# thomaspingel/neilpy

Hardware: AMD Instinct MI355X
Metric: Mcells/s through SMRF progressive_filter, 16384x16384 fp32 DEM (higher is better)
Workload: dtype f32

## Files before the change

### neilpy_amd/build.py

```python
import argparse
import os
import shutil
import subprocess
import sys
from concurrent.futures import ThreadPoolExecutor

PKG = os.path.dirname(os.path.abspath(__file__))
ROOT = os.path.dirname(PKG)
CSRC = os.path.join(PKG, "csrc")
OBJ = os.path.join(PKG, "_build")
LIBDIR = os.path.join(PKG, "_lib")
LIB = os.path.join(LIBDIR, "libsmrf_hip.so")
RING_PARTS = 8

FLAGS = ["-std=c++20", "-O3", "--offload-arch=gfx950", "-fPIC", "-ffp-contract=off",
         "-fvisibility=hidden", "-Wall", "-Wno-unused-function",
         "-I" + os.path.join(ROOT, "include"), "-I" + CSRC]


def hipcc():
    exe = shutil.which("hipcc") or "/opt/rocm/bin/hipcc"
    if not os.path.exists(exe):
        raise RuntimeError("hipcc not found: libsmrf_hip cannot be built (there is no CPU fallback)")
    return exe


def units():
    out = [(n + ".o", os.path.join(CSRC, n + ".hip"), []) for n in ("core", "morph", "incero", "chain", "grid", "springs", "fda", "tail", "spline", "terrain", "surface", "nearest", "focal", "morphometry", "points", "voxel", "relief", "assign", "footprint", "rank", "label")]
    for f64 in (0, 1):
        for p in range(RING_PARTS):
            out.append(("ring_%s_p%d.o" % ("f64" if f64 else "f32", p), os.path.join(CSRC, "ring_part.hip"),
                        ["-DPART=%d" % p, "-DSMRF_F64=%d" % f64]))
    return out


def newest_header():
    inc = os.path.join(ROOT, "include")
    t = max(os.path.getmtime(os.path.join(inc, f)) for f in os.listdir(inc) if f.endswith(".h"))
    for f in os.listdir(CSRC):
        if f.endswith((".h", ".inc")):
            t = max(t, os.path.getmtime(os.path.join(CSRC, f)))
    return t


def build(jobs=None, force=False, verbose=True, variant=None, defs=()):
    global OBJ, LIB
    if variant:
        OBJ = os.path.join(PKG, "_build", "variant_" + variant)
        LIB = os.path.join(LIBDIR, "variants", variant + ".so")
        os.makedirs(os.path.dirname(LIB), exist_ok=True)
    os.makedirs(OBJ, exist_ok=True)
    os.makedirs(LIBDIR, exist_ok=True)
    cc = hipcc()
    hdr = newest_header()
    todo = []
    objs = []
    for name, src, extra in units():
        obj = os.path.join(OBJ, name)
        objs.append(obj)
        if force or not os.path.exists(obj) or os.path.getmtime(obj) < max(os.path.getmtime(src), hdr):
            todo.append((obj, src, extra))

    def compile_one(job):
        obj, src, extra = job
        cmd = [cc] + FLAGS + list(defs) + extra + ["-c", src, "-o", obj]
        r = subprocess.run(cmd, capture_output=True, text=True)
        if r.returncode != 0:
            raise RuntimeError("hipcc failed: %s\n%s" % (" ".join(cmd), r.stderr[-4000:]))
        if verbose:
            print("  built", os.path.basename(obj), flush=True)
        return obj

    jobs = jobs or min(8, os.cpu_count() or 1)
    if todo:
        if verbose:
            print("compiling %d translation units for gfx950 with %d jobs" % (len(todo), jobs), flush=True)
        with ThreadPoolExecutor(max_workers=jobs) as ex:
            list(ex.map(compile_one, todo))
    if todo or not os.path.exists(LIB):
        cmd = [cc, "-shared", "-fPIC", "--offload-arch=gfx950", "-o", LIB] + objs
        r = subprocess.run(cmd, capture_output=True, text=True)
        if r.returncode != 0:
            raise RuntimeError("link failed: %s\n%s" % (" ".join(cmd), r.stderr[-4000:]))
        if verbose:
            print("linked", LIB, flush=True)
    return LIB


if __name__ == "__main__":
    ap = argparse.ArgumentParser()
    ap.add_argument("-j", type=int, default=None)
    ap.add_argument("--force", action="store_true")
    ap.add_argument("--variant", default=None)
    ap.add_argument("--defs", default="", help="extra compiler flags for a variant build, space separated")
    a = ap.parse_args()
    build(a.j, a.force, variant=a.variant, defs=tuple(a.defs.split()))
    sys.exit(0)
```

### neilpy_amd/csrc/core.hip

```cpp
#include <atomic>
#include <cstring>

#include "smrf_common.h"

namespace {
thread_local char g_err[512] = "";
}

namespace {
int env_int(const char* name, int dflt) {
  const char* v = getenv(name);
  return v && *v ? atoi(v) : dflt;
}
SmrfSwitches read_switches() {
  SmrfSwitches s;
  s.fused = env_int("SMRF_FUSED", 1);
  s.chain = env_int("SMRF_CHAIN", 1);
  s.nan_ride = env_int("SMRF_NAN_RIDE", 1);
  s.nt = env_int("SMRF_NT", -1);
  s.ring_seg = env_int("SMRF_RING_SEG", 0);
  s.ring_dual = env_int("SMRF_RING_DUAL", -1);
  s.ring_rounds = env_int("SMRF_RING_ROUNDS", 1);
  s.ring_slope = env_int("SMRF_RING_SLOPE", -1);
  s.seg_rule = env_int("SMRF_SEG_RULE", 0);
  s.xcd_remap = env_int("SMRF_XCD_REMAP", 1);
  s.fused_rounds = env_int("SMRF_FUSED_ROUNDS", 1);
  s.chain_rounds = env_int("SMRF_CHAIN_ROUNDS", 3);
  s.ring_debug = env_int("SMRF_RING_DEBUG", 0);
  s.ero_inc = env_int("SMRF_ERO_INC", 1);
  s.dil_cross = env_int("SMRF_DIL_CROSS", 1);
  return s;
}
std::atomic<const SmrfSwitches*> g_sw{new SmrfSwitches(read_switches())};
}

const SmrfSwitches& smrf_sw() { return *g_sw.load(std::memory_order_acquire); }

int smrf_fail(int code, const char* fmt, ...) {
  va_list ap;
  va_start(ap, fmt);
  vsnprintf(g_err, sizeof(g_err), fmt, ap);
  va_end(ap);
  return code;
}

extern "C" {

int smrf_abi_version(void) { return SMRF_ABI_VERSION; }

const char* smrf_last_error(void) { return g_err; }

void smrf_switches_reload(void) { g_sw.store(new SmrfSwitches(read_switches()), std::memory_order_release); }

int smrf_device_count(void) {
  int n = 0;
  if (hipGetDeviceCount(&n) != hipSuccess) {
    (void)hipGetLastError();
    return 0;
  }
  return n;
}

}
```

### neilpy_amd/csrc/morph.hip

```cpp
#include <algorithm>
#include <cmath>
#include <cstdlib>
#include <cstring>
#include <vector>

#include "smrf_common.h"
#include "morph_chain.h"

namespace {

template <typename T, bool DIL>
__global__ __launch_bounds__(256) void direct_kernel(const DiskArgs<T> a) {
  const int x = blockIdx.x * 64 + (threadIdx.x & 63);
  const int y = a.out_row0 + blockIdx.y * 4 + (threadIdx.x >> 6);
  if (x >= a.cols || y >= a.out_row0 + a.out_rows) return;
  const int r = a.radius;
  const long long r2 = (long long)r * r;
  T best = DIL ? -INFINITY : INFINITY;
  bool first_nan = false;
  for (int dy = -r; dy <= r; ++dy) {
    const int ly = smrf_fold(y + dy, a.img_rows) - a.in_row0;
    const T* row = a.in + (long long)ly * a.ld;
    long long rem = r2 - (long long)dy * dy;
    int w = (int)sqrt((double)rem);
    while ((long long)(w + 1) * (w + 1) <= rem) ++w;
    while ((long long)w * w > rem) --w;
    for (int dx = -w; dx <= w; ++dx) {
      const T v = row[smrf_fold(x + dx, a.cols)];
      if (dy == -r && dx == 0) first_nan = (v != v);
      if (DIL) { if (v > best) best = v; } else { if (v < best) best = v; }
    }
  }
  if (a.nan_aware && first_nan) best = DIL ? (T)NAN : (T)NAN;
  const long long off = (long long)(y - a.out_row0) * a.ld + x;
  a.out[off] = best;
  if (a.mask != nullptr) smrf::smrf_flag_cell(a, off, a.last[off], best);
}

template <typename T>
__global__ __launch_bounds__(256) void copy_flag_kernel(const DiskArgs<T> a) {
  const long long n = (long long)a.out_rows * a.cols;
  for (long long i = blockIdx.x * 256ll + threadIdx.x; i < n; i += (long long)gridDim.x * 256) {
    const int yy = (int)(i / a.cols), x = (int)(i % a.cols);
    const T v = a.in[(long long)(a.out_row0 + yy - a.in_row0) * a.ld + x];
    const long long off = (long long)yy * a.ld + x;
    a.out[off] = v;
    if (a.mask != nullptr) smrf::smrf_flag_cell(a, off, a.last[off], v);
  }
}

template <typename T>
__global__ __launch_bounds__(256) void count_nan_kernel(const T* __restrict__ p, long long n,
                                                        unsigned long long* __restrict__ out) {
  unsigned long long c = 0;
  for (long long i = blockIdx.x * 256ll + threadIdx.x; i < n; i += (long long)gridDim.x * 256) {
    const T v = p[i];
    c += (v != v);
  }
  for (int o = 32; o > 0; o >>= 1) c += __shfl_down(c, o, 64);
  if ((threadIdx.x & 63) == 0 && c) atomicAdd(out, c);
}

template <typename T> struct RingFn;
template <> struct RingFn<float> {
  static int call(const DiskArgs<float>& a, int d, hipStream_t s) {
    switch (a.radius % SMRF_RING_PARTS) {
      case 0: return smrf_ring_f32_p0(a, d, s);
      case 1: return smrf_ring_f32_p1(a, d, s);
      case 2: return smrf_ring_f32_p2(a, d, s);
      case 3: return smrf_ring_f32_p3(a, d, s);
      case 4: return smrf_ring_f32_p4(a, d, s);
      case 5: return smrf_ring_f32_p5(a, d, s);
      case 6: return smrf_ring_f32_p6(a, d, s);
      default: return smrf_ring_f32_p7(a, d, s);
    }
  }
};
template <> struct RingFn<double> {
  static int call(const DiskArgs<double>& a, int d, hipStream_t s) {
    switch (a.radius % SMRF_RING_PARTS) {
      case 0: return smrf_ring_f64_p0(a, d, s);
      case 1: return smrf_ring_f64_p1(a, d, s);
      case 2: return smrf_ring_f64_p2(a, d, s);
      case 3: return smrf_ring_f64_p3(a, d, s);
      case 4: return smrf_ring_f64_p4(a, d, s);
      case 5: return smrf_ring_f64_p5(a, d, s);
      case 6: return smrf_ring_f64_p6(a, d, s);
      default: return smrf_ring_f64_p7(a, d, s);
    }
  }
};

template <typename T>
int check_band(const DiskArgs<T>& a) {
  if (!a.in || !a.out) return smrf_fail(SMRF_E_ARG, "null raster pointer");
  if (a.img_rows < 1 || a.cols < 1 || a.in_rows < 1 || a.out_rows < 1 || a.radius < 0)
    return smrf_fail(SMRF_E_ARG, "bad raster size (%d x %d, in %d, out %d, radius %d)", a.img_rows,
                     a.cols, a.in_rows, a.out_rows, a.radius);
  if (a.ld < a.cols) return smrf_fail(SMRF_E_ARG, "ld %lld < cols %d", a.ld, a.cols);
  if (a.out_row0 < 0 || a.out_row0 + a.out_rows > a.img_rows || a.in_row0 < 0 ||
      a.in_row0 + a.in_rows > a.img_rows)
    return smrf_fail(SMRF_E_ARG, "row band outside the raster");
  const int lo = a.out_row0 - a.radius, hi = a.out_row0 + a.out_rows + a.radius;
  const int span = hi - lo;
  if (span >= 2 * a.img_rows) {
    if (a.in_row0 != 0 || a.in_rows != a.img_rows)
      return smrf_fail(SMRF_E_ARG, "band must hold the whole raster when radius >= rows");
  } else {
    for (int y = lo; y < hi; ++y) {
      const int g = smrf_fold(y, a.img_rows);
      if (g < a.in_row0 || g >= a.in_row0 + a.in_rows)
        return smrf_fail(SMRF_E_ARG, "input band [%d,%d) lacks row %d needed by output rows [%d,%d) at radius %d",
                         a.in_row0, a.in_row0 + a.in_rows, g, a.out_row0, a.out_row0 + a.out_rows, a.radius);
    }
  }
  return SMRF_OK;
}

template <typename T>
int disk_filter(DiskArgs<T> a, bool dilate, int impl, hipStream_t stream) {
  if (int rc = check_band(a)) return rc;
  if (a.radius == 0) {
    const long long n = (long long)a.out_rows * a.cols;
    const int blocks = (int)std::min<long long>((n + 255) / 256, 4096);
    hipLaunchKernelGGL(copy_flag_kernel<T>, dim3(blocks), dim3(256), 0, stream, a);
    SMRF_LAUNCH_CHECK();
    return SMRF_OK;
  }
  if (impl == SMRF_IMPL_AUTO) impl = a.radius <= SMRF_RING_MAX_RADIUS ? SMRF_IMPL_RING : SMRF_IMPL_DIRECT;
  if (impl == SMRF_IMPL_RING) {
    if (a.radius > SMRF_RING_MAX_RADIUS)
      return smrf_fail(SMRF_E_UNSUPPORTED, "ring kernels cover radius <= %d (got %d)", SMRF_RING_MAX_RADIUS, a.radius);
    a.seg = smrf_sw().ring_seg;
    return RingFn<T>::call(a, dilate ? SMRF_RING_DILATE : SMRF_RING_ERODE, stream);
  }
  if (impl != SMRF_IMPL_DIRECT) return smrf_fail(SMRF_E_ARG, "unknown impl %d", impl);
  dim3 grid((a.cols + 63) / 64, (a.out_rows + 3) / 4);
  if (dilate) hipLaunchKernelGGL((direct_kernel<T, true>), grid, dim3(256), 0, stream, a);
  else hipLaunchKernelGGL((direct_kernel<T, false>), grid, dim3(256), 0, stream, a);
  SMRF_LAUNCH_CHECK();
  return SMRF_OK;
}

template <typename T>
int nt_rule(int img_rows, int cols) {
  const int env = smrf_sw().nt;
  if (env >= 0) return env != 0;
  return (size_t)img_rows * (size_t)cols * sizeof(T) >= ((size_t)192 << 20);
}

template <typename T, template <typename> class Args>
void set_band(Args<T>& a, int img_rows, int cols, int64_t ld, int in_row0, int in_rows, int out_row0, int out_rows) {
  a.img_rows = img_rows; a.cols = cols; a.ld = ld;
  a.in_row0 = in_row0; a.in_rows = in_rows; a.out_row0 = out_row0; a.out_rows = out_rows;
  a.nt = nt_rule<T>(img_rows, cols);
}

template <typename T>
int disk_filter_api(const T* in, T* out, int img_rows, int cols, int64_t ld, int in_row0, int in_rows,
                    int out_row0, int out_rows, int radius, int is_dilate, int nan_aware, int impl, void* stream) {
  DiskArgs<T> a{};
  a.in = in; a.out = out;
  set_band(a, img_rows, cols, ld, in_row0, in_rows, out_row0, out_rows);
  a.radius = radius; a.nan_aware = nan_aware;
  return disk_filter(a, is_dilate != 0, impl, (hipStream_t)stream);
}

template <typename T>
int dilate_flag_api(const T* eroded, const T* last, T* opened, uint8_t* mask, uint8_t* when, double thr,
                    int widx, int img_rows, int cols, int64_t ld, int in_row0, int in_rows, int out_row0,
                    int out_rows, int radius, int nan_aware, int impl, void* stream, int dense = 0) {
  if (!last || !mask) return smrf_fail(SMRF_E_ARG, "null last/mask pointer");
  DiskArgs<T> a{};
  a.in = eroded; a.out = opened; a.last = last; a.mask = mask; a.when = when; a.thr = thr; a.thr_lo = smrf_float_below(thr); a.widx = widx;
  set_band(a, img_rows, cols, ld, in_row0, in_rows, out_row0, out_rows);
  a.radius = radius; a.nan_aware = nan_aware; a.dense = dense;
  return disk_filter(a, true, impl, (hipStream_t)stream);
}

int dilate_cross_flag_f32(const float* e_prev, const float* last, float* opened, uint8_t* mask, uint8_t* when, double thr, int widx,
                          int rows, int cols, int radius, hipStream_t stream) {
  if (!smrf_dil_cross_has(4, radius)) return smrf_fail(SMRF_E_UNSUPPORTED, "no cross-on-load dilation for radius %d", radius);
  DiskArgs<float> a{};
  a.in = e_prev; a.out = opened; a.last = last; a.mask = mask; a.when = when; a.thr = thr; a.thr_lo = smrf_float_below(thr); a.widx = widx;
  set_band(a, rows, cols, cols, 0, rows, 0, rows);
  a.radius = radius;
  if (int rc = check_band(a)) return rc;
  a.seg = smrf_sw().ring_seg;
  return RingFn<float>::call(a, SMRF_RING_DILATE_CROSS, stream);
}

template <typename T>
int count_nan_api(const T* p, int64_t n, int64_t* h_count, void* stream_) {
  hipStream_t stream = (hipStream_t)stream_;
  if (!h_count || (n > 0 && !p)) return smrf_fail(SMRF_E_ARG, "null pointer");
  *h_count = 0;
  if (n <= 0) return SMRF_OK;
  unsigned long long* d = nullptr;
  SMRF_HIP_CHECK(hipMallocAsync((void**)&d, sizeof(*d), stream));
  SMRF_HIP_CHECK(hipMemsetAsync(d, 0, sizeof(*d), stream));
  const int blocks = (int)std::min<long long>((n + 255) / 256, 2048);
  hipLaunchKernelGGL(count_nan_kernel<T>, dim3(blocks), dim3(256), 0, stream, p, (long long)n, d);
  unsigned long long h = 0;
  hipError_t e = hipMemcpyAsync(&h, d, sizeof(h), hipMemcpyDeviceToHost, stream);
  if (e == hipSuccess) e = hipStreamSynchronize(stream);
  hipFreeAsync(d, stream);
  SMRF_HIP_CHECK(e);
  *h_count = (int64_t)h;
  return SMRF_OK;
}

template <typename T>
int open_flag_api(const T* last, T* opened, uint8_t* mask, uint8_t* when, double thr, int widx, int img_rows, int cols,
                  int64_t ld, int in_row0, int in_rows, int out_row0, int out_rows, int radius, void* stream, int dense = 0) {
  if (!smrf_fused_radius((int)sizeof(T), radius))
    return smrf_fail(SMRF_E_UNSUPPORTED, "no fused opening kernel for radius %d at this dtype", radius);
  DiskArgs<T> a{};
  a.in = last; a.out = opened; a.mask = mask; a.when = when; a.thr = thr; a.thr_lo = smrf_float_below(thr); a.widx = widx;
  set_band(a, img_rows, cols, ld, in_row0, in_rows, out_row0, out_rows);
  a.radius = 2 * radius;
  if (int rc = check_band(a)) return rc;
  a.radius = radius;
  a.last = last + (long long)(out_row0 - in_row0) * ld;
  a.nan_aware = 0;
  a.dense = mask ? dense : 0;
  a.seg = smrf_sw().ring_seg;
  return RingFn<T>::call(a, SMRF_RING_FUSED_OPEN, (hipStream_t)stream);
}

template <typename T>
int chain_launch(int pat, ChainArgs<T> c, int img_rows, int cols, int64_t ld, int in_row0, int in_rows, int out_row0, int out_rows,
                 hipStream_t stream) {
  set_band(c, img_rows, cols, ld, in_row0, in_rows, out_row0, out_rows);
  c.seg = smrf_sw().ring_seg;
  if constexpr (sizeof(T) == 4) return smrf_chain_f32(pat, c, stream);
  else return smrf_chain_f64(pat, c, stream);
}

template <typename T>
int chain_flag_api(const T* last, T* opened, uint8_t* mask, uint8_t* when, const int32_t* radii, const double* thr,
                   const int32_t* widx, int n, int img_rows, int cols, int64_t ld, int in_row0, int in_rows, int out_row0,
                   int out_rows, void* stream) {
  if (!last || !opened || !mask || !radii || !thr || !widx) return smrf_fail(SMRF_E_ARG, "null pointer");
  if (n < 1 || n > 4) return smrf_fail(SMRF_E_ARG, "a chain has 1..4 windows (got %d)", n);
  const int pat = smrf_chain_match((int)sizeof(T), radii, n, kPfAnySize);
  if (pat < 0 || smrf_chain_length(pat) != n)
    return smrf_fail(SMRF_E_UNSUPPORTED, "no chained launch for these %d radii at this dtype (smrf_pf_chain_length tells)", n);
  DiskArgs<T> b{};
  b.in = last; b.out = opened;
  set_band(b, img_rows, cols, ld, in_row0, in_rows, out_row0, out_rows);
  b.radius = smrf_chain_halo(pat);
  if (int rc = check_band(b)) return rc;
  if (b.radius >= img_rows) return smrf_fail(SMRF_E_UNSUPPORTED, "raster of %d rows is shorter than the chain's %d halo rows", img_rows, b.radius);
  ChainArgs<T> c{};
  c.in = last; c.out = opened; c.mask = mask; c.when = when;
  for (int k = 0; k < n; ++k) { c.thr[k] = thr[k]; c.widx[k] = widx[k]; }
  return chain_launch(pat, c, img_rows, cols, ld, in_row0, in_rows, out_row0, out_rows, (hipStream_t)stream);
}

thread_local std::vector<uint8_t> g_ero_inc_taken;

template <typename T>
int progressive_filter_api(const T* Z, int rows, int cols, const int32_t* windows, const double* thr, int nwin,
                           uint8_t* mask, uint8_t* when, void* ws, size_t ws_bytes, int nan_aware, int impl,
                           void* stream_, float* h_window_ms = nullptr, int32_t* h_window_route = nullptr) {
  hipStream_t stream = (hipStream_t)stream_;
  if (!Z || !mask || (nwin > 0 && (!windows || !thr))) return smrf_fail(SMRF_E_ARG, "null pointer");
  if (rows < 1 || cols < 1 || nwin < 0) return smrf_fail(SMRF_E_ARG, "bad size");
  const size_t need = smrf_progressive_filter_workspace_bytes(rows, cols, (int)sizeof(T));
  if (ws_bytes < need || !ws) return smrf_fail(SMRF_E_WORKSPACE, "workspace %zu < %zu bytes", ws_bytes, need);
  for (int i = 0; i < nwin; ++i)
    if (windows[i] < 0) return smrf_fail(SMRF_E_ARG, "negative window %d", windows[i]);
  const size_t plane = (size_t)rows * cols;
  T* E = reinterpret_cast<T*>(ws);
  T* P[3] = {E, E + plane, E + 2 * plane};
  auto at = [&](int k) -> const T* { return k == kPfPlaneZ ? Z : P[k]; };
  if (nwin == 0) {
    SMRF_HIP_CHECK(hipMemsetAsync(mask, 0, plane, stream));
    if (when) SMRF_HIP_CHECK(hipMemsetAsync(when, 0, plane, stream));
  }
  const SmrfSwitches& sw = smrf_sw();
  SmrfPfRules rules{(int)sizeof(T), sw.fused, sw.chain, sw.ero_inc, impl, nan_aware > 0, 0, sw.dil_cross};
  std::vector<int32_t> plan_buf((size_t)2 * nwin);
  int32_t* const route = plan_buf.data();
  int32_t* const pattern = route + nwin;
  g_ero_inc_taken.assign((size_t)nwin, 0);
  std::vector<uint8_t> fold((size_t)nwin, 0);
  std::vector<SmrfPfStep> steps((size_t)2 * nwin);
  int nsteps = 0;
  auto make_plan = [&](int with_nan) {
    rules.nan_aware = with_nan;
    smrf_pf_route(rules, windows, nwin, rows, (long long)plane, route, g_ero_inc_taken.data(), pattern);
    smrf_pf_fold(rules, windows, route, g_ero_inc_taken.data(), nwin, fold.data());
    nsteps = smrf_pf_steps(windows, route, g_ero_inc_taken.data(), fold.data(), pattern, nwin, steps.data());
  };
  make_plan(nan_aware > 0);
  unsigned* d_nan = nullptr;
  if (nan_aware < 0) {
    if (nsteps > 0 && steps[0].kind == kPfStepChain && sw.nan_ride != 0) {
      d_nan = reinterpret_cast<unsigned*>(E);
      SMRF_HIP_CHECK(hipMemsetAsync(d_nan, 0, sizeof(unsigned), stream));
      nan_aware = 0;
    } else {
      int64_t c = 0;
      if (int rc = count_nan_api<T>(Z, (int64_t)plane, &c, stream_)) return rc;
      nan_aware = c > 0;
      if (nan_aware) make_plan(1);
    }
  }
  struct Events {
    std::vector<hipEvent_t> v;
    ~Events() { for (hipEvent_t e : v) if (e) hipEventDestroy(e); }
  } evs;
  std::vector<hipEvent_t>& ev = evs.v;
  if (h_window_ms) {
    ev.assign((size_t)nwin + 1, nullptr);
    for (auto& e : ev) SMRF_HIP_CHECK(hipEventCreate(&e));
    SMRF_HIP_CHECK(hipEventRecord(ev[0], stream));
  }
  auto window_done = [&](int i) -> int {
    if (h_window_route) h_window_route[i] = route[i];
    if (h_window_ms) SMRF_HIP_CHECK(hipEventRecord(ev[(size_t)i + 1], stream));
    return SMRF_OK;
  };
  auto finish = [&]() -> int {
    if (!h_window_ms) return SMRF_OK;
    hipError_t e = nwin > 0 ? hipEventSynchronize(ev[(size_t)nwin]) : hipSuccess;
    for (int i = 0; i < nwin && e == hipSuccess; ++i) e = hipEventElapsedTime(&h_window_ms[i], ev[(size_t)i], ev[(size_t)i + 1]);
    SMRF_HIP_CHECK(e);
    return SMRF_OK;
  };
  for (int s = 0; s < nsteps;) {
    const SmrfPfStep& st = steps[(size_t)s];
    const int i = st.win, r = windows[i];
    T* const dst = P[st.dst];
    switch (st.kind) {
      case kPfStepChain: {
        ChainArgs<T> c{};
        c.in = at(st.src); c.out = dst; c.mask = mask; c.when = when;
        for (int k = 0; k < st.len; ++k) { c.thr[k] = thr[i + k]; c.widx[k] = i + k; }
        c.dense0 = st.dense;
        c.nan_flag = d_nan;
        if (int rc = chain_launch(st.pattern, c, rows, cols, cols, 0, rows, 0, rows, stream)) return rc;
        if (d_nan) {
          unsigned h = 0;
          SMRF_HIP_CHECK(hipMemcpyAsync(&h, d_nan, sizeof(h), hipMemcpyDeviceToHost, stream));
          SMRF_HIP_CHECK(hipStreamSynchronize(stream));
          d_nan = nullptr;
          if (h) {
            nan_aware = 1;
            make_plan(1);
            continue;
          }
        }
        break;
      }
      case kPfStepFused:
        if (int rc = open_flag_api<T>(at(st.src), dst, mask, when, thr[i], i, rows, cols, cols, 0, rows, 0, rows, r, stream_, st.dense)) return rc;
        break;
      case kPfStepErode:
        if (int rc = disk_filter_api<T>(at(st.src), dst, rows, cols, cols, 0, rows, 0, rows, r, 0, nan_aware, impl, stream_)) return rc;
        break;
      case kPfStepIncErode:
        if constexpr (sizeof(T) == 4) {
          if (int rc = smrf_inc_erode_f32(at(st.src), at(st.aux), dst, rows, cols, cols, r, nt_rule<T>(rows, cols), stream)) return rc;
          break;
        } else {
          return smrf_fail(SMRF_E_HIP, "internal: no incremental erosion at this dtype");
        }
      case kPfStepDilate:
        if (int rc = dilate_flag_api<T>(at(st.src), at(st.aux), dst, mask, when, thr[i], i, rows, cols, cols, 0, rows, 0, rows, r,
                                        nan_aware, impl, stream_, st.dense))
          return rc;
        break;
      case kPfStepDilateCross:
        if constexpr (sizeof(T) == 4) {
          if (int rc = dilate_cross_flag_f32(at(st.src), at(st.aux), dst, mask, when, thr[i], i, rows, cols, r, stream)) return rc;
          break;
        } else {
          return smrf_fail(SMRF_E_HIP, "internal: no cross on load at this dtype");
        }
      default:
        return smrf_fail(SMRF_E_HIP, "internal: unknown step kind %d", st.kind);
    }
    if (st.closes)
      for (int k = 0; k < st.len; ++k)
        if (int rc = window_done(i + k)) return rc;
    ++s;
  }
  return finish();
}

}

extern "C" {

int smrf_disk_filter_f32(const float* d_in, float* d_out, int img_rows, int cols, int64_t ld, int in_row0,
                         int in_rows, int out_row0, int out_rows, int radius, int is_dilate, int nan_aware,
                         int impl, void* stream) {
  return disk_filter_api<float>(d_in, d_out, img_rows, cols, ld, in_row0, in_rows, out_row0, out_rows, radius,
                                is_dilate, nan_aware, impl, stream);
}
int smrf_disk_filter_f64(const double* d_in, double* d_out, int img_rows, int cols, int64_t ld, int in_row0,
                         int in_rows, int out_row0, int out_rows, int radius, int is_dilate, int nan_aware,
                         int impl, void* stream) {
  return disk_filter_api<double>(d_in, d_out, img_rows, cols, ld, in_row0, in_rows, out_row0, out_rows, radius,
                                 is_dilate, nan_aware, impl, stream);
}
int smrf_pf_dilate_flag_f32(const float* d_eroded, const float* d_last, float* d_opened, uint8_t* d_mask,
                            uint8_t* d_when_dropped, double threshold, int window_index, int img_rows, int cols,
                            int64_t ld, int in_row0, int in_rows, int out_row0, int out_rows, int radius,
                            int nan_aware, int impl, void* stream) {
  return dilate_flag_api<float>(d_eroded, d_last, d_opened, d_mask, d_when_dropped, threshold, window_index,
                                img_rows, cols, ld, in_row0, in_rows, out_row0, out_rows, radius, nan_aware, impl,
                                stream);
}
int smrf_pf_dilate_flag_f64(const double* d_eroded, const double* d_last, double* d_opened, uint8_t* d_mask,
                            uint8_t* d_when_dropped, double threshold, int window_index, int img_rows, int cols,
                            int64_t ld, int in_row0, int in_rows, int out_row0, int out_rows, int radius,
                            int nan_aware, int impl, void* stream) {
  return dilate_flag_api<double>(d_eroded, d_last, d_opened, d_mask, d_when_dropped, threshold, window_index,
                                 img_rows, cols, ld, in_row0, in_rows, out_row0, out_rows, radius, nan_aware, impl,
                                 stream);
}
int smrf_fused_open_supported(int elem_size, int radius) { return smrf_fused_radius(elem_size, radius) ? 1 : 0; }
int smrf_pf_open_flag_f32(const float* d_last, float* d_opened, uint8_t* d_mask, uint8_t* d_when_dropped, double threshold,
                          int window_index, int img_rows, int cols, int64_t ld, int in_row0, int in_rows, int out_row0,
                          int out_rows, int radius, void* stream) {
  if (!d_last || !d_opened) return smrf_fail(SMRF_E_ARG, "null raster pointer");
  return open_flag_api<float>(d_last, d_opened, d_mask, d_when_dropped, threshold, window_index, img_rows, cols, ld, in_row0,
                              in_rows, out_row0, out_rows, radius, stream);
}
int smrf_pf_open_flag_f64(const double* d_last, double* d_opened, uint8_t* d_mask, uint8_t* d_when_dropped, double threshold,
                          int window_index, int img_rows, int cols, int64_t ld, int in_row0, int in_rows, int out_row0,
                          int out_rows, int radius, void* stream) {
  if (!d_last || !d_opened) return smrf_fail(SMRF_E_ARG, "null raster pointer");
  return open_flag_api<double>(d_last, d_opened, d_mask, d_when_dropped, threshold, window_index, img_rows, cols, ld, in_row0,
                               in_rows, out_row0, out_rows, radius, stream);
}
int smrf_pf_chain_length(int elem_size, const int32_t* h_radii, int n, int64_t raster_cells) {
  if (!h_radii || n < 1) return 0;
  const SmrfSwitches& sw = smrf_sw();
  if (sw.chain == 0 || sw.fused == 0) return 0;
  const int pat = smrf_chain_match(elem_size, h_radii, n, sw.fused == 2 ? kPfAnySize : (long long)raster_cells);
  return pat < 0 ? 0 : smrf_chain_length(pat);
}
int smrf_pf_plan(int elem_size, const int32_t* h_windows, int n, int rows, int64_t cells, int nan_aware, int impl, int band,
                 int32_t* h_route, uint8_t* h_ero_inc) {
  if (n < 0 || (n > 0 && (!h_windows || !h_route || !h_ero_inc))) return smrf_fail(SMRF_E_ARG, "null pointer");
  if ((elem_size != 4 && elem_size != 8) || rows < 1 || cells < 0 || band < 0 || band > 2)
    return smrf_fail(SMRF_E_ARG, "bad plan question (element size %d, %d rows, band %d)", elem_size, rows, band);
  for (int i = 0; i < n; ++i)
    if (h_windows[i] < 0) return smrf_fail(SMRF_E_ARG, "negative window %d", h_windows[i]);
  const SmrfSwitches& sw = smrf_sw();
  smrf_pf_route(SmrfPfRules{elem_size, sw.fused, sw.chain, sw.ero_inc, impl, nan_aware != 0, band}, h_windows, n, rows,
                (long long)cells, h_route, h_ero_inc);
  return SMRF_OK;
}
int smrf_pf_chain_flag_f32(const float* d_last, float* d_opened, uint8_t* d_mask, uint8_t* d_when_dropped,
                           const int32_t* h_radii, const double* h_thresholds, const int32_t* h_window_index, int n_windows,
                           int img_rows, int cols, int64_t ld, int in_row0, int in_rows, int out_row0, int out_rows,
                           void* stream) {
  return chain_flag_api<float>(d_last, d_opened, d_mask, d_when_dropped, h_radii, h_thresholds, h_window_index, n_windows,
                               img_rows, cols, ld, in_row0, in_rows, out_row0, out_rows, stream);
}
int smrf_pf_chain_flag_f64(const double* d_last, double* d_opened, uint8_t* d_mask, uint8_t* d_when_dropped,
                           const int32_t* h_radii, const double* h_thresholds, const int32_t* h_window_index, int n_windows,
                           int img_rows, int cols, int64_t ld, int in_row0, int in_rows, int out_row0, int out_rows,
                           void* stream) {
  return chain_flag_api<double>(d_last, d_opened, d_mask, d_when_dropped, h_radii, h_thresholds, h_window_index, n_windows,
                                img_rows, cols, ld, in_row0, in_rows, out_row0, out_rows, stream);
}
int smrf_pf_ero_inc_windows(uint8_t* h_taken, int n) {
  if (!h_taken || n < 0) return smrf_fail(SMRF_E_ARG, "null h_taken");
  const int have = (int)g_ero_inc_taken.size();
  for (int i = 0; i < n; ++i) h_taken[i] = i < have ? g_ero_inc_taken[(size_t)i] : 0;
  return have;
}
size_t smrf_progressive_filter_workspace_bytes(int rows, int cols, int elem_size) {
  return (size_t)3 * (size_t)rows * (size_t)cols * (size_t)elem_size;
}
int smrf_progressive_filter_f32(const float* d_Z, int rows, int cols, const int32_t* h_windows,
                                const double* h_thresholds, int n_windows, uint8_t* d_mask, uint8_t* d_when_dropped,
                                void* d_workspace, size_t workspace_bytes, int nan_aware, int impl, void* stream) {
  return progressive_filter_api<float>(d_Z, rows, cols, h_windows, h_thresholds, n_windows, d_mask, d_when_dropped,
                                       d_workspace, workspace_bytes, nan_aware, impl, stream);
}
int smrf_progressive_filter_f64(const double* d_Z, int rows, int cols, const int32_t* h_windows,
                                const double* h_thresholds, int n_windows, uint8_t* d_mask, uint8_t* d_when_dropped,
                                void* d_workspace, size_t workspace_bytes, int nan_aware, int impl, void* stream) {
  return progressive_filter_api<double>(d_Z, rows, cols, h_windows, h_thresholds, n_windows, d_mask, d_when_dropped,
                                        d_workspace, workspace_bytes, nan_aware, impl, stream);
}
int smrf_progressive_filter_timed_f32(const float* d_Z, int rows, int cols, const int32_t* h_windows,
                                      const double* h_thresholds, int n_windows, uint8_t* d_mask, uint8_t* d_when_dropped,
                                      void* d_workspace, size_t workspace_bytes, int nan_aware, int impl, void* stream,
                                      float* h_window_ms, int32_t* h_window_route) {
  if (!h_window_ms) return smrf_fail(SMRF_E_ARG, "null h_window_ms");
  return progressive_filter_api<float>(d_Z, rows, cols, h_windows, h_thresholds, n_windows, d_mask, d_when_dropped,
                                       d_workspace, workspace_bytes, nan_aware, impl, stream, h_window_ms, h_window_route);
}
int smrf_progressive_filter_timed_f64(const double* d_Z, int rows, int cols, const int32_t* h_windows,
                                      const double* h_thresholds, int n_windows, uint8_t* d_mask, uint8_t* d_when_dropped,
                                      void* d_workspace, size_t workspace_bytes, int nan_aware, int impl, void* stream,
                                      float* h_window_ms, int32_t* h_window_route) {
  if (!h_window_ms) return smrf_fail(SMRF_E_ARG, "null h_window_ms");
  return progressive_filter_api<double>(d_Z, rows, cols, h_windows, h_thresholds, n_windows, d_mask, d_when_dropped,
                                        d_workspace, workspace_bytes, nan_aware, impl, stream, h_window_ms, h_window_route);
}
int smrf_count_nan_f32(const float* d_a, int64_t n, int64_t* h_count, void* stream) {
  return count_nan_api<float>(d_a, n, h_count, stream);
}
int smrf_count_nan_f64(const double* d_a, int64_t n, int64_t* h_count, void* stream) {
  return count_nan_api<double>(d_a, n, h_count, stream);
}

}
```

### neilpy_amd/csrc/morph_chain.h

```cpp
#pragma once
#include "morph_ring.h"

template <typename T>
struct ChainArgs {
  const T* in;
  T* out;
  uint8_t* mask;
  uint8_t* when;
  double thr[4];
  float thr_lo[4];
  int widx[4];
  int img_rows, cols;
  long long ld;
  int in_row0, in_rows, out_row0, out_rows;
  int seg;
  int nt;
  int dense0;
  unsigned* nan_flag;
};

SMRF_HIDDEN int smrf_chain_f32(int pattern, const ChainArgs<float>& a, hipStream_t s);
SMRF_HIDDEN int smrf_chain_f64(int pattern, const ChainArgs<double>& a, hipStream_t s);

#ifndef SMRF_CHAIN_NP_ALL
#define SMRF_CHAIN_NP_ALL 0
#endif
#ifndef SMRF_CHAIN_NP
#define SMRF_CHAIN_NP(T, PAT) (SMRF_CHAIN_NP_ALL ? SMRF_CHAIN_NP_ALL : (sizeof(T) == 4 ? ((PAT) <= 2 || (PAT) == 8 ? 4 : 3) : 1))
#endif

namespace smrf {

template <int NP_, int R0, int R1, int R2, int R3>
struct ChainCfg {
  static constexpr int NP = NP_, ROWS = 2 * NP_, TW = 256;
  static constexpr int NW = (R0 > 0) + (R1 > 0) + (R2 > 0) + (R3 > 0);
  static constexpr int radius(int i) { return i == 0 ? R0 : i == 1 ? R1 : i == 2 ? R2 : R3; }
  static constexpr int RM = R3 > 0 ? R3 : R2 > 0 ? R2 : R1 > 0 ? R1 : R0;
  static constexpr int delay(int i) {
    int d = 0;
    for (int j = 0; j <= i; ++j) d += 2 * radius(j);
    return d;
  }
  static constexpr int S = delay(NW - 1);
  static constexpr int TWO = TW - 2 * S;
  static constexpr int kq(int i) { return (2 * radius(i) + ROWS - 1) / ROWS; }
  static constexpr int KQM = (2 * RM + ROWS - 1) / ROWS;
  static constexpr int WB = TW + 2 * RM;
  static constexpr int BUF = NP * WB;
  static constexpr int CELLS = 2 * BUF;
};

#ifndef SMRF_CHAIN_GROUP
#define SMRF_CHAIN_GROUP(T, R) chain_group<T>(R)
#endif
template <typename T> constexpr int chain_group(int r) { return sizeof(T) == 4 ? (r >= 11 ? 4 : 0) : (r >= 4 ? 2 : 0); }

template <typename T, int R, bool DIL, int NP, int WB, int NACC, int G>
__device__ __forceinline__ void chain_stage_grouped(typename Vec2<T>::type* const buf, const int tid, T (&acc)[NACC],
                                                    typename Vec2<T>::type (&io)[NP]) {
  using S = DiskShape<R>;
  using T2 = typename Vec2<T>::type;
  static_assert(NACC >= 2 * R && G >= 1, "ring too short / no group size");
  constexpr int K = S::K, KR1 = S::kidx(R - 1);
  constexpr int NGR = (R + G - 1) / G;
  constexpr int NQ = NP * NGR;
  const unsigned base = (unsigned)(size_t)(__attribute__((address_space(3))) void*)(buf + tid);
  T2 lft[2][G], rgt[2][G];
  auto issue = [&]<int Q>(std::integral_constant<int, Q>) {
    constexpr int P = Q / NGR, c0 = (Q % NGR) * G;
    [&]<int... Cc>(std::integer_sequence<int, Cc...>) {
      (([&] {
         if constexpr (c0 + Cc < R) {
           lft[Q & 1][Cc] = lds_read2<(P * WB + R - 1 - (c0 + Cc)) * (int)sizeof(T2)>(base, T());
           rgt[Q & 1][Cc] = lds_read2<(P * WB + R + 1 + (c0 + Cc)) * (int)sizeof(T2)>(base, T());
         }
       }()), ...);
    }(std::make_integer_sequence<int, G>{});
  };
  issue(std::integral_constant<int, 0>{});
  auto pair_body = [&]<int P>(std::integral_constant<int, P>) {
       T ra[K], rb[K];
       ra[0] = io[P].x;
       rb[0] = io[P].y;
       T a = ra[0], b = rb[0];
       [&]<int... Gi>(std::integer_sequence<int, Gi...>) {
         (([&] {
            constexpr int Q = P * NGR + Gi, c0 = Gi * G;
            if constexpr (Q + 1 < NQ) {
              constexpr int nxt = ((Q + 1) % NGR + 1) * G <= R ? G : R - ((Q + 1) % NGR) * G;
              issue(std::integral_constant<int, Q + 1>{});
              lds_wait<2 * nxt>();
            } else {
              lds_wait<0>();
            }
            [&]<int... Cc>(std::integer_sequence<int, Cc...>) {
              (([&] {
                 constexpr int c = c0 + Cc;
                 if constexpr (c < R) {
                   a = op3<DIL>(a, lft[Q & 1][Cc].x, rgt[Q & 1][Cc].x);
                   b = op3<DIL>(b, lft[Q & 1][Cc].y, rgt[Q & 1][Cc].y);
                   [&]<int... Kk>(std::integer_sequence<int, Kk...>) {
                     (([&] { if constexpr (S::wk(Kk + 1) == c + 1) { ra[Kk + 1] = a; rb[Kk + 1] = b; } }()), ...);
                   }(std::make_integer_sequence<int, K - 1>{});
                 }
               }()), ...);
            }(std::make_integer_sequence<int, G>{});
          }()), ...);
       }(std::make_integer_sequence<int, NGR>{});
       const T o0 = op2<DIL>(acc[0], ra[0]);
       const T o1 = op3<DIL>(acc[1], ra[KR1], rb[0]);
       [&]<int... Sl>(std::integer_sequence<int, Sl...>) {
         (([&] {
            constexpr int da = R - Sl - 2 < 0 ? -(R - Sl - 2) : R - Sl - 2, db = R - Sl - 1 < 0 ? -(R - Sl - 1) : R - Sl - 1;
            acc[Sl] = op3<DIL>(acc[Sl + 2], ra[S::kidx(da)], rb[S::kidx(db)]);
          }()), ...);
       }(std::make_integer_sequence<int, 2 * R - 2>{});
       acc[2 * R - 2] = op2<DIL>(ra[0], rb[KR1]);
       acc[2 * R - 1] = rb[0];
       io[P].x = o0;
       io[P].y = o1;
  };
  [&]<int... P>(std::integer_sequence<int, P...>) {
    (pair_body(std::integral_constant<int, P>{}), ...);
  }(std::make_integer_sequence<int, NP>{});
}

template <typename T, int R, bool DIL, int NP, int WB, int NACC>
__device__ __forceinline__ void chain_stage(typename Vec2<T>::type* const buf, const int tid, T (&acc)[NACC],
                                            typename Vec2<T>::type (&io)[NP]) {
  using S = DiskShape<R>;
  using T2 = typename Vec2<T>::type;
  static_assert(NACC >= 2 * R, "ring too short");
  if constexpr (SMRF_CHAIN_GROUP(T, R) > 0) {
    chain_stage_grouped<T, R, DIL, NP, WB, NACC, SMRF_CHAIN_GROUP(T, R)>(buf, tid, acc, io);
    return;
  }
  constexpr int K = S::K, KR1 = S::kidx(R - 1);
  constexpr bool AHEAD = R <= 4 && NP > 1;
  const unsigned base = (unsigned)(size_t)(__attribute__((address_space(3))) void*)(buf + tid);
  T2 lft[AHEAD ? 2 : 1][R], rgt[AHEAD ? 2 : 1][R];
  auto issue = [&]<int P>(std::integral_constant<int, P>) {
    [&]<int... Cc>(std::integer_sequence<int, Cc...>) {
      ((lft[AHEAD ? (P & 1) : 0][Cc] = lds_read2<(P * WB + R - 1 - Cc) * (int)sizeof(T2)>(base, T()),
        rgt[AHEAD ? (P & 1) : 0][Cc] = lds_read2<(P * WB + R + 1 + Cc) * (int)sizeof(T2)>(base, T())), ...);
    }(std::make_integer_sequence<int, R>{});
  };
  if constexpr (AHEAD) issue(std::integral_constant<int, 0>{});
  [&]<int... P>(std::integer_sequence<int, P...>) {
    (([&] {
       constexpr int B = AHEAD ? (P & 1) : 0;
       if constexpr (AHEAD && P + 1 < NP) {
         issue(std::integral_constant<int, P + 1>{});
         lds_wait<2 * R>();
       } else {
         if constexpr (!AHEAD) issue(std::integral_constant<int, P>{});
         lds_wait<0>();
       }
       T ra[K], rb[K];
       ra[0] = io[P].x;
       rb[0] = io[P].y;
       [&]<int... Kk>(std::integer_sequence<int, Kk...>) {
         (([&] {
            constexpr int k = Kk + 1;
            T a = ra[k - 1], b = rb[k - 1];
#pragma unroll
            for (int c = S::wk(k - 1); c < S::wk(k); ++c) {
              a = op3<DIL>(a, lft[B][c].x, rgt[B][c].x);
              b = op3<DIL>(b, lft[B][c].y, rgt[B][c].y);
            }
            ra[k] = a;
            rb[k] = b;
          }()), ...);
       }(std::make_integer_sequence<int, K - 1>{});
       const T o0 = op2<DIL>(acc[0], ra[0]);
       const T o1 = op3<DIL>(acc[1], ra[KR1], rb[0]);
       [&]<int... Sl>(std::integer_sequence<int, Sl...>) {
         (([&] {
            constexpr int da = R - Sl - 2 < 0 ? -(R - Sl - 2) : R - Sl - 2, db = R - Sl - 1 < 0 ? -(R - Sl - 1) : R - Sl - 1;
            acc[Sl] = op3<DIL>(acc[Sl + 2], ra[S::kidx(da)], rb[S::kidx(db)]);
          }()), ...);
       }(std::make_integer_sequence<int, 2 * R - 2>{});
       acc[2 * R - 2] = op2<DIL>(ra[0], rb[KR1]);
       acc[2 * R - 1] = rb[0];
       io[P].x = o0;
       io[P].y = o1;
     }()), ...);
  }(std::make_integer_sequence<int, NP>{});
}

template <typename T, int NP, int OCC, int R0, int R1, int R2, int R3>
__global__ __launch_bounds__(256, OCC)
void chain_kernel(const ChainArgs<T> a) {
  using C = ChainCfg<NP, R0, R1, R2, R3>;
  using T2 = typename Vec2<T>::type;
  constexpr int NW = C::NW, ROWS = C::ROWS, TW = C::TW, S = C::S, TWO = C::TWO, RM = C::RM, KQM = C::KQM;
  static_assert(TWO >= 64, "chain too long for a 256-column strip");
  extern __shared__ __attribute__((aligned(16))) unsigned char smrf_lds[];
  T2* const L = reinterpret_cast<T2*>(smrf_lds);

  const int tid = threadIdx.x;
  const int xe0 = (int)blockIdx.x * TWO - S;
  const int x = xe0 + tid;
  const bool owns = tid >= S && tid < TW - S && x < a.cols;
  const int cx = smrf_fold(x, a.cols);
  const int ys = a.out_row0 + (int)blockIdx.y * a.seg;
  const int ye = min(a.out_row0 + a.out_rows, ys + a.seg);
  const int last_in = a.in_rows - 1;
  const bool flag = a.mask != nullptr;
  float thr_lo[NW];
#pragma unroll
  for (int i = 0; i < NW; ++i) thr_lo[i] = a.thr_lo[i];

  T accE[NW][2 * RM], accD[NW][2 * RM];
#pragma unroll
  for (int i = 0; i < NW; ++i)
#pragma unroll
    for (int s = 0; s < 2 * RM; ++s) { accE[i][s] = ident<T>(false); accD[i][s] = ident<T>(true); }
  T2 dq[NW][KQM][NP];
#pragma unroll
  for (int i = 0; i < NW; ++i)
#pragma unroll
    for (int s = 0; s < KQM; ++s)
#pragma unroll
      for (int p = 0; p < NP; ++p) { dq[i][s][p].x = T(0); dq[i][s][p].y = T(0); }
  T2 pf[NP];
  T outv[ROWS];
  bool hit[NW][ROWS];
#pragma unroll
  for (int r = 0; r < ROWS; ++r) {
    outv[r] = T(0);
#pragma unroll
    for (int i = 0; i < NW; ++i) hit[i][r] = false;
  }

  constexpr int DELTA = (ROWS - (2 * S) % ROWS) % ROWS;
  const int ystart = ys - S - DELTA;
  RowFold rf(ystart, a.img_rows);
  auto prefetch = [&]() {
    const int l0 = rf.p - a.in_row0;
    if (rf.p + ROWS <= rf.n && l0 >= 0 && l0 + ROWS - 1 <= last_in) {
      const T* r0 = a.in + (long long)l0 * a.ld + cx;
#pragma unroll
      for (int p = 0; p < NP; ++p) {
        pf[p].x = r0[(long long)(2 * p) * a.ld];
        pf[p].y = r0[(long long)(2 * p + 1) * a.ld];
      }
    } else {
#pragma unroll
      for (int p = 0; p < NP; ++p) {
        int la = rf.at(2 * p) - a.in_row0;
        int lb = rf.at(2 * p + 1) - a.in_row0;
        la = la < 0 ? 0 : (la > last_in ? last_in : la);
        lb = lb < 0 ? 0 : (lb > last_in ? last_in : lb);
        pf[p].x = a.in[(long long)la * a.ld + cx];
        pf[p].y = a.in[(long long)lb * a.ld + cx];
      }
    }
    rf.advance(ROWS);
  };
  auto epilogue = [&](int yyb) {
    if (!owns) return;
    [&]<int... I>(std::integer_sequence<int, I...>) {
      (([&] {
         if (flag) {
           const int y0 = yyb - C::delay(I);
           const bool dense = I == 0 && a.dense0;
           const long long off0 = (long long)(y0 - a.out_row0) * a.ld + x;
           if (y0 >= ys && y0 + ROWS <= ye && !dense) {
             bool any = false;
#pragma unroll
             for (int r = 0; r < ROWS; ++r) any = any || hit[I][r];
             if (any) {
#pragma unroll
               for (int r = 0; r < ROWS; ++r)
                 if (hit[I][r]) {
                   a.mask[off0 + (long long)r * a.ld] = 1;
                   if (a.when != nullptr) a.when[off0 + (long long)r * a.ld] = (uint8_t)a.widx[I];
                 }
             }
           } else {
#pragma unroll
             for (int r = 0; r < ROWS; ++r) {
               const int y = y0 + r;
               if (y >= ys && y < ye) {
                 const long long off = off0 + (long long)r * a.ld;
                 if (dense) {
                   a.mask[off] = hit[I][r] ? 1 : 0;
                   if (a.when != nullptr) a.when[off] = hit[I][r] ? (uint8_t)a.widx[I] : (uint8_t)0;
                 } else if (hit[I][r]) {
                   a.mask[off] = 1;
                   if (a.when != nullptr) a.when[off] = (uint8_t)a.widx[I];
                 }
               }
             }
           }
         }
       }()), ...);
    }(std::make_integer_sequence<int, NW>{});
    const int yob = yyb - S;
    if (yob >= ys) {
      const long long off0 = (long long)(yob - a.out_row0) * a.ld + x;
      if (yob + ROWS <= ye) {
        if (a.nt) {
#pragma unroll
          for (int r = 0; r < ROWS; ++r) __builtin_nontemporal_store(outv[r], &a.out[off0 + (long long)r * a.ld]);
        } else {
#pragma unroll
          for (int r = 0; r < ROWS; ++r) a.out[off0 + (long long)r * a.ld] = outv[r];
        }
      } else {
#pragma unroll
        for (int r = 0; r < ROWS; ++r)
          if (yob + r < ye) smrf_store_out(&a.out[off0 + (long long)r * a.ld], outv[r], a.nt);
      }
    }
  };

  const bool scan = a.nan_flag != nullptr;
  bool seen_nan = false;
  prefetch();
  for (int yy0 = ystart; yy0 < ye + S; yy0 += ROWS) {
    T2 cur[NP];
#pragma unroll
    for (int p = 0; p < NP; ++p) cur[p] = pf[p];
    if (scan) {
#pragma unroll
      for (int p = 0; p < NP; ++p) seen_nan = seen_nan || cur[p].x != cur[p].x || cur[p].y != cur[p].y;
    }
    if (yy0 > ystart) epilogue(yy0 - ROWS);
    if (yy0 + ROWS < ye + S) prefetch();
    [&]<int... I>(std::integer_sequence<int, I...>) {
      (([&] {
         constexpr int R = C::radius(I), KQ = C::kq(I), WB = C::WB;
         T2* const bufE = L;
         T2* const bufD = L + C::BUF;
         T lastv[ROWS];
#pragma unroll
         for (int r = 0; r < ROWS; ++r) {
           const int e = r - 2 * R + KQ * ROWS, slot = e / ROWS, w = e % ROWS;
           const T2 src = slot < KQ ? dq[I][slot < KQ ? slot : 0][w / 2] : cur[w / 2];
           lastv[r] = (w & 1) ? src.y : src.x;
         }
#pragma unroll
         for (int sl = 0; sl + 1 < KQ; ++sl)
#pragma unroll
           for (int p = 0; p < NP; ++p) dq[I][sl][p] = dq[I][sl + 1][p];
#pragma unroll
         for (int p = 0; p < NP; ++p) dq[I][KQ - 1][p] = cur[p];
#pragma unroll
         for (int p = 0; p < NP; ++p)
           lds_write2((unsigned)(size_t)(__attribute__((address_space(3))) void*)(bufE + p * WB + R + tid), cur[p]);
         lds_wait<0>();
         __syncthreads();
         chain_stage<T, R, false, NP, WB>(bufE, tid, accE[I], cur);
#pragma unroll
         for (int p = 0; p < NP; ++p)
           lds_write2((unsigned)(size_t)(__attribute__((address_space(3))) void*)(bufD + p * WB + R + tid), cur[p]);
         lds_wait<0>();
         __syncthreads();
         chain_stage<T, R, true, NP, WB>(bufD, tid, accD[I], cur);
#pragma unroll
         for (int r = 0; r < ROWS; ++r) {
           const T opened = (r & 1) ? cur[r / 2].y : cur[r / 2].x;
           const T diff = lastv[r] - opened;
           if constexpr (sizeof(T) == 4) hit[I][r] = diff > thr_lo[I];
           else hit[I][r] = (double)diff > a.thr[I];
         }
       }()), ...);
    }(std::make_integer_sequence<int, NW>{});
#pragma unroll
    for (int r = 0; r < ROWS; ++r) outv[r] = (r & 1) ? cur[r / 2].y : cur[r / 2].x;
  }
  {
    const int nb = (ye + S - ystart + ROWS - 1) / ROWS;
    epilogue(ystart + (nb - 1) * ROWS);
  }
  if (scan && seen_nan) atomicOr(a.nan_flag, 1u);
}

template <typename T, int NP, int OCC, int R0, int R1, int R2, int R3>
int chain_launch(const ChainArgs<T>& a_in, hipStream_t stream) {
  using C = ChainCfg<NP, R0, R1, R2, R3>;
  using T2 = typename Vec2<T>::type;
  constexpr size_t LDS = (size_t)C::CELLS * sizeof(T2);
  constexpr auto kern = chain_kernel<T, NP, OCC, R0, R1, R2, R3>;
  int resident;
  bool first;
  if (int rc = smrf_resident<kern>(C::TW, LDS, resident, first)) return rc;
  if (first && smrf_sw().ring_debug)
    fprintf(stderr, "smrf chain: R=%d,%d,%d,%d %s NP=%d LDS=%zu, %d workgroups/CU resident\n", R0, R1, R2, R3,
            sizeof(T) == 4 ? "f32" : "f64", NP, LDS, resident);
  ChainArgs<T> a = a_in;
  const int strips = (a.cols + C::TWO - 1) / C::TWO;
  a.seg = smrf_seg_len(a.out_rows, strips, resident, smrf_sw().chain_rounds, 2 * C::S, C::ROWS, std::max(32, 4 * C::S),
                       smrf_sw().seg_rule, a.seg);
  dim3 grid(strips, (a.out_rows + a.seg - 1) / a.seg);
  hipLaunchKernelGGL(kern, grid, dim3(C::TW), LDS, stream, a);
  SMRF_LAUNCH_CHECK();
  return SMRF_OK;
}

}
```

### neilpy_amd/csrc/pf_route.h

```cpp
#pragma once
#include <cstdint>

constexpr int kPfImplAuto = 0, kPfImplRing = 1, kPfImplDirect = 2, kPfRingMaxRadius = 64;
constexpr int kPfRouteTwoPass = 0, kPfRouteFused = 1, kPfRouteDirect = 2, kPfRouteCopy = 3, kPfRouteChain = 4;
#ifdef SMRF_HIP_H
static_assert(kPfImplAuto == SMRF_IMPL_AUTO && kPfImplRing == SMRF_IMPL_RING && kPfImplDirect == SMRF_IMPL_DIRECT &&
              kPfRingMaxRadius == SMRF_RING_MAX_RADIUS && kPfRouteTwoPass == SMRF_ROUTE_TWO_PASS &&
              kPfRouteFused == SMRF_ROUTE_FUSED && kPfRouteDirect == SMRF_ROUTE_DIRECT && kPfRouteCopy == SMRF_ROUTE_COPY &&
              kPfRouteChain == SMRF_ROUTE_CHAIN, "pf_route.h restates include/smrf_hip.h");
#endif

struct SmrfChainPattern { int n; int r[4]; long long min_cells; long long min_cells_f64; };
constexpr long long kLarge = 20ll << 20;
constexpr long long kMid = 16ll << 20;
constexpr long long kSmall = 4ll << 20;
constexpr long long kNever = -1;
constexpr SmrfChainPattern kPatterns[] = {{3, {1, 2, 3, 0}, 0, 0}, {2, {1, 2, 0, 0}, 0, 0}, {2, {2, 3, 0, 0}, 0, 0}, {2, {4, 5, 0, 0}, kLarge, kNever},
                                          {1, {4, 0, 0, 0}, 0, 0}, {1, {5, 0, 0, 0}, 0, 0}, {1, {6, 0, 0, 0}, 0, kNever}, {1, {7, 0, 0, 0}, 0, kSmall},
                                          {1, {8, 0, 0, 0}, 0, kMid}, {1, {9, 0, 0, 0}, 0, kNever}, {1, {10, 0, 0, 0}, kLarge, kNever}};
constexpr int kNPatterns = (int)(sizeof(kPatterns) / sizeof(kPatterns[0]));
constexpr long long kPfAnySize = 1ll << 62;

inline int smrf_chain_match(int elem_size, const int32_t* windows, int n, long long cells) {
  for (int p = 0; p < kNPatterns; ++p) {
    const long long mc = elem_size == 8 ? kPatterns[p].min_cells_f64 : kPatterns[p].min_cells;
    if (kPatterns[p].n > n || mc < 0 || cells < mc) continue;
    bool ok = true;
    for (int i = 0; i < kPatterns[p].n; ++i) ok = ok && windows[i] == kPatterns[p].r[i];
    if (ok) return p;
  }
  return -1;
}
inline int smrf_chain_length(int pat) { return pat >= 0 && pat < kNPatterns ? kPatterns[pat].n : 0; }
inline int smrf_chain_halo(int pat) {
  int s = 0;
  if (pat >= 0 && pat < kNPatterns)
    for (int i = 0; i < kPatterns[pat].n; ++i) s += 2 * kPatterns[pat].r[i];
  return s;
}

#ifndef SMRF_FUSED_MAX_RADIUS
#define SMRF_FUSED_MAX_RADIUS 14
#endif
constexpr bool smrf_fused_radius(int elem_size, int r) {
  if (r < 1 || r > SMRF_FUSED_MAX_RADIUS) return false;
  return elem_size == 4 ? (r != 9) : (r <= 6);
}
constexpr int kFusedSmallRadius = 8;
constexpr long long kFusedLargeCells = 20ll << 20;

#define SMRF_INCERO_MIN_RADIUS 16
#define SMRF_INCERO_MAX_RADIUS 64
namespace smrf {
#include "ero_inc_adopt.inc"
}
inline bool smrf_inc_erode_has(int elem_size, int radius) {
  return elem_size == 4 && radius >= SMRF_INCERO_MIN_RADIUS && radius <= SMRF_INCERO_MAX_RADIUS;
}
inline bool smrf_inc_erode_adopted(int elem_size, int radius) {
  return smrf_inc_erode_has(elem_size, radius) && smrf::kEroIncAdoptF32[radius] != 0;
}

constexpr bool smrf_dil_cross_has(int elem_size, int radius) {
  return elem_size == 4 && (radius == 16 || radius == 21 || radius == 36);
}
namespace smrf {
#include "dil_cross_adopt.inc"
}
inline bool smrf_dil_cross_adopted(int elem_size, int radius) {
  return smrf_dil_cross_has(elem_size, radius) && smrf::kDilCrossAdoptF32[radius] != 0;
}

struct SmrfPfRules {
  int elem_size;
  int fused;
  int chain;
  int ero_inc;
  int impl;
  int nan_aware;
  int band;
  int dil_cross;
};

inline void smrf_pf_route(const SmrfPfRules& k, const int32_t* windows, int n, int rows, long long cells, int32_t* route,
                          uint8_t* ero_inc, int32_t* pattern = nullptr) {
  const bool fuse_ok = !k.nan_aware && (k.impl == kPfImplAuto || k.impl == kPfImplRing) && k.fused != 0;
  const bool chain_ok = fuse_ok && k.chain != 0 && k.band != 2;
  for (int i = 0; i < n; ++i) {
    ero_inc[i] = 0;
    if (pattern) pattern[i] = -1;
  }
  for (int i = 0; i < n;) {
    const int r = windows[i];
    const int pat = chain_ok ? smrf_chain_match(k.elem_size, windows + i, n - i, k.fused == 2 ? kPfAnySize : cells) : -1;
    const int len = pat >= 0 && smrf_chain_halo(pat) < rows ? smrf_chain_length(pat) : 0;
    if (len) {
      if (pattern) pattern[i] = pat;
      for (int j = 0; j < len; ++j) route[i + j] = kPfRouteChain + j;
      i += len;
      continue;
    }
    if (fuse_ok && smrf_fused_radius(k.elem_size, r) &&
        (r <= kFusedSmallRadius || (!k.band && (k.fused == 2 || cells >= kFusedLargeCells)))) {
      route[i++] = kPfRouteFused;
      continue;
    }
    const int eff = k.impl == kPfImplAuto ? (r <= kPfRingMaxRadius ? kPfImplRing : kPfImplDirect) : k.impl;
    route[i] = r == 0 ? kPfRouteCopy : eff == kPfImplRing ? kPfRouteTwoPass : kPfRouteDirect;
    ero_inc[i] = !k.band && k.ero_inc != 0 && !k.nan_aware && i > 0 && route[i] == kPfRouteTwoPass &&
                 route[i - 1] == kPfRouteTwoPass && r == windows[i - 1] + 1 && smrf_inc_erode_has(k.elem_size, r) &&
                 (k.ero_inc == 2 || smrf_inc_erode_adopted(k.elem_size, r));
    ++i;
  }
}

constexpr uint8_t kPfFoldNone = 0, kPfFoldCross = 1, kPfFoldAfter = 2;
inline void smrf_pf_fold(const SmrfPfRules& k, const int32_t* windows, const int32_t* route, const uint8_t* ero_inc, int n,
                         uint8_t* fold) {
  (void)ero_inc;
  const bool ok = k.dil_cross != 0 && !k.band && !k.nan_aware && k.elem_size == 4 && (k.impl == kPfImplAuto || k.impl == kPfImplRing);
  for (int i = 0; i < n; ++i) {
    fold[i] = i > 0 && fold[i - 1] == kPfFoldCross ? kPfFoldAfter : kPfFoldNone;
    if (!ok || i == 0 || fold[i] != kPfFoldNone) continue;
    const int r = windows[i];
    if (route[i] != kPfRouteTwoPass || route[i - 1] != kPfRouteTwoPass || r != windows[i - 1] + 1 || !smrf_dil_cross_has(k.elem_size, r))
      continue;
    if (k.dil_cross == 2 || (smrf_dil_cross_adopted(k.elem_size, r) && i + 1 < n)) fold[i] = kPfFoldCross;
  }
}
inline bool smrf_pf_runs_inc(const uint8_t* ero_inc, const uint8_t* fold, int i) { return ero_inc[i] != 0 && fold[i] == kPfFoldNone; }

constexpr int kPfStepChain = 0, kPfStepFused = 1, kPfStepErode = 2, kPfStepIncErode = 3, kPfStepDilate = 4, kPfStepDilateCross = 5;
constexpr int kPfPlaneZ = -1, kPfPlaneNone = -2;
struct SmrfPfStep { int kind, win, len, src, aux, dst, dense, closes, pattern; };

inline int smrf_pf_steps(const int32_t* windows, const int32_t* route, const uint8_t* ero_inc, const uint8_t* fold,
                         const int32_t* pattern, int n, SmrfPfStep* steps) {
  (void)windows;
  int pe = 0, pl = kPfPlaneZ, m = 0;
  for (int i = 0; i < n;) {
    int po = 0;
    while (po == pe || po == pl) ++po;
    int len = 1;
    if (route[i] == kPfRouteChain) {
      len = smrf_chain_length(pattern[i]);
      steps[m++] = {kPfStepChain, i, len, pl, kPfPlaneNone, po, i == 0, 1, pattern[i]};
      pl = po;
    } else if (route[i] == kPfRouteFused) {
      steps[m++] = {kPfStepFused, i, 1, pl, kPfPlaneNone, po, i == 0, 1, -1};
      pl = po;
    } else if (fold[i] == kPfFoldCross) {
      steps[m++] = {kPfStepDilateCross, i, 1, pe, pl, po, 0, 1, -1};
      pl = po;
    } else if (smrf_pf_runs_inc(ero_inc, fold, i)) {
      steps[m++] = {kPfStepIncErode, i, 1, pe, pl, po, 0, 0, -1};
      steps[m++] = {kPfStepDilate, i, 1, po, pl, pe, 0, 1, -1};
      pl = pe;
      pe = po;
    } else {
      steps[m++] = {kPfStepErode, i, 1, pl, kPfPlaneNone, pe, 0, 0, -1};
      steps[m++] = {kPfStepDilate, i, 1, pe, pl, po, i == 0, 1, -1};
      pl = po;
    }
    i += len;
  }
  return m;
}
```

### neilpy_amd/csrc/smrf_common.h

```cpp
#pragma once
#include <hip/hip_runtime.h>
#include <cstdarg>
#include <cstdint>
#include <cstdio>
#include <cstdlib>
#include <algorithm>

#include "smrf_hip.h"

#define SMRF_HIDDEN __attribute__((visibility("hidden")))

SMRF_HIDDEN int smrf_fail(int code, const char* fmt, ...) __attribute__((format(printf, 2, 3)));

#define SMRF_HIP_CHECK(expr)                                                                  \
  do {                                                                                        \
    hipError_t e_ = (expr);                                                                   \
    if (e_ != hipSuccess)                                                                     \
      return smrf_fail(SMRF_E_HIP, "%s failed: %s (%s:%d)", #expr, hipGetErrorString(e_),     \
                       __FILE__, __LINE__);                                                   \
  } while (0)

#define SMRF_LAUNCH_CHECK() SMRF_HIP_CHECK(hipGetLastError())

__host__ __device__ inline int smrf_fold(int i, int n) {
  const int p2 = 2 * n;
  int p = i % p2;
  if (p < 0) p += p2;
  return p < n ? p : p2 - 1 - p;
}

template <typename F>
__device__ __forceinline__ void smrf_xcd_tile(const bool plain, F&& general_allowed, int& bx, int& by) {
  bx = blockIdx.x;
  by = blockIdx.y;
  if (plain) {
  } else if ((gridDim.x & 7) == 0) {
    const int id = blockIdx.y * gridDim.x + blockIdx.x, per = gridDim.x >> 3;
    const int xcd = id & 7, slot = id >> 3;
    bx = xcd * per + slot % per;
    by = slot / per;
  } else if (gridDim.x > 8 && general_allowed()) {
    const int total = gridDim.x * gridDim.y, id = blockIdx.y * gridDim.x + blockIdx.x;
    const int xcd = id & 7, slot = id >> 3, q = total >> 3, rem = total & 7;
    const int t = xcd * q + (xcd < rem ? xcd : rem) + slot;
    bx = t / (int)gridDim.y;
    by = t % (int)gridDim.y;
  }
}

struct SmrfSwitches {
  int fused;
  int chain;
  int nan_ride;
  int nt;
  int ring_seg;
  int ring_dual;
  int ring_rounds, fused_rounds, chain_rounds;
  int seg_rule;
  int xcd_remap;
  int ring_slope;
  int ring_debug;
  int ero_inc;
  int dil_cross;
};
SMRF_HIDDEN const SmrfSwitches& smrf_sw();

inline int smrf_blocks(long long n, int cap) { return (int)std::max<long long>(1, std::min<long long>((n + 255) / 256, cap)); }

inline size_t smrf_up256(size_t bytes) { return (bytes + 255) & ~(size_t)255; }

__host__ __device__ constexpr int smrf_isqrt(int v) {
  int r = 0;
  while ((long long)(r + 1) * (r + 1) <= v) ++r;
  return r;
}

inline float smrf_float_below(double t) {
  float f = (float)t;
  if ((double)f > t) f = __builtin_nextafterf(f, -__builtin_inff());
  return f;
}

#include "seg_rule.h"
#include "pf_route.h"

template <auto Kern>
int smrf_resident(int block, size_t lds, int& resident, bool& first) {
  static int resident_of[64] = {0};
  int dev = 0;
  SMRF_HIP_CHECK(hipGetDevice(&dev));
  if (dev < 0 || dev >= 64) return smrf_fail(SMRF_E_UNSUPPORTED, "device index %d out of range", dev);
  resident = __atomic_load_n(&resident_of[dev], __ATOMIC_ACQUIRE);
  first = resident == 0;
  if (first) {
    const void* const kern = reinterpret_cast<const void*>(Kern);
    if (lds > 48 * 1024) SMRF_HIP_CHECK(hipFuncSetAttribute(kern, hipFuncAttributeMaxDynamicSharedMemorySize, (int)lds));
    int nb = 0;
    SMRF_HIP_CHECK(hipOccupancyMaxActiveBlocksPerMultiprocessor(&nb, kern, block, lds));
    resident = std::max(1, nb);
    __atomic_store_n(&resident_of[dev], resident, __ATOMIC_RELEASE);
  }
  return SMRF_OK;
}

template <typename T>
struct DiskArgs {
  const T* in;
  T* out;
  const T* last;
  uint8_t* mask;
  uint8_t* when;
  double thr;
  float thr_lo;
  int widx;
  int img_rows, cols;
  long long ld;
  int in_row0, in_rows, out_row0, out_rows;
  int radius;
  int nan_aware;
  int seg;
  int nt;
  int dense;
  int seg_cls;
  int seg_first[8], seg_row0[8], seg_len[8];
  int plain_tiles;
};

enum { SMRF_RING_ERODE = 0, SMRF_RING_DILATE = 1, SMRF_RING_FUSED_OPEN = 2, SMRF_RING_DILATE_CROSS = 3 };
SMRF_HIDDEN int smrf_inc_erode_f32(const float* e_prev, const float* last, float* out, int rows, int cols, long long ld,
                                   int radius, int nt, hipStream_t s);
#define SMRF_RING_PARTS 8
#define SMRF_RING_DECL(P)                                                                     \
  SMRF_HIDDEN int smrf_ring_f32_p##P(const DiskArgs<float>&, int mode, hipStream_t);          \
  SMRF_HIDDEN int smrf_ring_f64_p##P(const DiskArgs<double>&, int mode, hipStream_t);
SMRF_RING_DECL(0) SMRF_RING_DECL(1) SMRF_RING_DECL(2) SMRF_RING_DECL(3)
SMRF_RING_DECL(4) SMRF_RING_DECL(5) SMRF_RING_DECL(6) SMRF_RING_DECL(7)
#undef SMRF_RING_DECL
```

Before: 4378.

## Add cross-stage chained kernels that derive consecutive-radius openings from previous erosion

Adds a chained morphology kernel variant in which, for consecutive window radii r and r+1, a stage's erosion is computed from the previous stage's eroded result using a small cross (plus-shaped) structuring element instead of a full disk. The planner matches fixed radius runs ({5,6,7}, {6,7}, {1,2,3}) and routes them to this kernel for f32 when the input is not NaN-aware and is not banded. This is meant to cut the per-row LDS reduction work and the halo for small-radius chains. It relies on static asserts that these disk radii decompose exactly, and it adds a new kernel instantiation with its own occupancy and register pressure.

```diff
diff --git a/include/smrf_small_cross.h b/include/smrf_small_cross.h
--- /dev/null
+++ b/include/smrf_small_cross.h
@@ -0,0 +1,18 @@
+#ifndef SMRF_SMALL_CROSS_H
+#define SMRF_SMALL_CROSS_H
+
+#include "smrf_hip.h"
+
+#ifdef __cplusplus
+extern "C" {
+#endif
+
+SMRF_API int smrf_pf_small_cross_windows(uint8_t* h_taken, int n);
+SMRF_API int smrf_pf_small_cross_plan(int elem_size, const int32_t* h_windows, int n, int rows, int64_t cells, int nan_aware,
+                                      int impl, int band, uint8_t* h_small);
+
+#ifdef __cplusplus
+}
+#endif
+
+#endif
diff --git a/neilpy_amd/build.py b/neilpy_amd/build.py
--- a/neilpy_amd/build.py
+++ b/neilpy_amd/build.py
@@ -26,7 +26,7 @@
 
 
 def units():
-    out = [(n + ".o", os.path.join(CSRC, n + ".hip"), []) for n in ("core", "morph", "incero", "chain", "grid", "springs", "fda", "tail", "spline", "terrain", "surface", "nearest", "focal", "morphometry", "points", "voxel", "relief", "assign", "footprint", "rank", "label")]
+    out = [(n + ".o", os.path.join(CSRC, n + ".hip"), []) for n in ("core", "morph", "incero", "chain", "chain_cross", "grid", "springs", "fda", "tail", "spline", "terrain", "surface", "nearest", "focal", "morphometry", "points", "voxel", "relief", "assign", "footprint", "rank", "label")]
     for f64 in (0, 1):
         for p in range(RING_PARTS):
             out.append(("ring_%s_p%d.o" % ("f64" if f64 else "f32", p), os.path.join(CSRC, "ring_part.hip"),
diff --git a/neilpy_amd/csrc/chain_cross.hip b/neilpy_amd/csrc/chain_cross.hip
--- /dev/null
+++ b/neilpy_amd/csrc/chain_cross.hip
@@ -0,0 +1,42 @@
+#include "morph_chain.h"
+
+namespace {
+
+#ifndef SMRF_XCHAIN_NP
+#define SMRF_XCHAIN_NP(XPAT) ((XPAT) == 2 ? 4 : (XPAT) == 1 ? 2 : 3)
+#endif
+#ifndef SMRF_XCHAIN_OCC
+#define SMRF_XCHAIN_OCC(XPAT) ((XPAT) == 0 ? 3 : 4)
+#endif
+namespace rim {
+#include "ero_inc.inc"
+}
+constexpr bool cross_patterns_are_rim_free() {
+  for (int p = 0; p < kNCrossPatterns; ++p)
+    for (int i = 0; i < kCrossPatterns[p].n; ++i)
+      if ((kCrossPatterns[p].cross >> i) & 1u)
+        if (i == 0 || kCrossPatterns[p].r[i] != kCrossPatterns[p].r[i - 1] + 1 || rim::kEroInc[kCrossPatterns[p].r[i]].n != 0) return false;
+  return true;
+}
+static_assert(cross_patterns_are_rim_free(), "kCrossPatterns (pf_route.h) against ero_inc.inc");
+template <int XPAT>
+int launch_cross(const ChainArgs<float>& a, hipStream_t s) {
+  constexpr SmrfCrossPattern p = kCrossPatterns[XPAT];
+  static_assert(smrf::ChainCfg<SMRF_XCHAIN_NP(XPAT), p.r[0], p.r[1], p.r[2], p.r[3], p.cross>::S == p.halo, "kCrossPatterns: halo");
+  return smrf::chain_launch<float, SMRF_XCHAIN_NP(XPAT), SMRF_XCHAIN_OCC(XPAT), p.r[0], p.r[1], p.r[2], p.r[3], p.cross>(a, s);
+}
+
+}
+
+int smrf_chain_cross_f32(int xpat, const ChainArgs<float>& a_in, hipStream_t s) {
+  static_assert(kNCrossPatterns == 3, "one case per row of kCrossPatterns");
+  ChainArgs<float> a = a_in;
+  for (int i = 0; i < 4; ++i) a.thr_lo[i] = smrf_float_below(a.thr[i]);
+  switch (xpat) {
+    case 0: return launch_cross<0>(a, s);
+    case 1: return launch_cross<1>(a, s);
+    case 2: return launch_cross<2>(a, s);
+    default: break;
+  }
+  return smrf_fail(SMRF_E_ARG, "no cross-stage chain kernel for pattern %d", xpat);
+}
diff --git a/neilpy_amd/csrc/chain_kernel_body.inc b/neilpy_amd/csrc/chain_kernel_body.inc
--- /dev/null
+++ b/neilpy_amd/csrc/chain_kernel_body.inc
@@ -0,0 +1,208 @@
+  using T2 = typename Vec2<T>::type;
+  constexpr int NW = C::NW, ROWS = C::ROWS, TW = C::TW, S = C::S, TWO = C::TWO, RM = C::RM, KQM = C::KQM;
+  static_assert(TWO >= 64, "chain too long for a 256-column strip");
+  static_assert(C::valid(), "a cross stage needs a window before it in the chain");
+  extern __shared__ __attribute__((aligned(16))) unsigned char smrf_lds[];
+  T2* const L = reinterpret_cast<T2*>(smrf_lds);
+
+  const int tid = threadIdx.x;
+  const int xe0 = (int)blockIdx.x * TWO - S;
+  const int x = xe0 + tid;
+  const bool owns = tid >= S && tid < TW - S && x < a.cols;
+  const int cx = smrf_fold(x, a.cols);
+  const int ys = a.out_row0 + (int)blockIdx.y * a.seg;
+  const int ye = min(a.out_row0 + a.out_rows, ys + a.seg);
+  const int last_in = a.in_rows - 1;
+  const bool flag = a.mask != nullptr;
+  float thr_lo[NW];
+#pragma unroll
+  for (int i = 0; i < NW; ++i) thr_lo[i] = a.thr_lo[i];
+
+  T accE[NW][2 * RM], accD[NW][2 * RM];
+#pragma unroll
+  for (int i = 0; i < NW; ++i)
+#pragma unroll
+    for (int s = 0; s < 2 * RM; ++s) { accE[i][s] = ident<T>(false); accD[i][s] = ident<T>(true); }
+  T xc[NW][3];
+#pragma unroll
+  for (int i = 0; i < NW; ++i)
+#pragma unroll
+    for (int s = 0; s < 3; ++s) xc[i][s] = ident<T>(false);
+  T2 dq[NW][KQM][NP];
+#pragma unroll
+  for (int i = 0; i < NW; ++i)
+#pragma unroll
+    for (int s = 0; s < KQM; ++s)
+#pragma unroll
+      for (int p = 0; p < NP; ++p) { dq[i][s][p].x = T(0); dq[i][s][p].y = T(0); }
+  T2 pf[NP];
+  T outv[ROWS];
+  bool hit[NW][ROWS];
+#pragma unroll
+  for (int r = 0; r < ROWS; ++r) {
+    outv[r] = T(0);
+#pragma unroll
+    for (int i = 0; i < NW; ++i) hit[i][r] = false;
+  }
+
+  constexpr int DELTA = (ROWS - (2 * S) % ROWS) % ROWS;
+  const int ystart = ys - S - DELTA;
+  RowFold rf(ystart, a.img_rows);
+  auto prefetch = [&]() {
+    const int l0 = rf.p - a.in_row0;
+    if (rf.p + ROWS <= rf.n && l0 >= 0 && l0 + ROWS - 1 <= last_in) {
+      const T* r0 = a.in + (long long)l0 * a.ld + cx;
+#pragma unroll
+      for (int p = 0; p < NP; ++p) {
+        pf[p].x = r0[(long long)(2 * p) * a.ld];
+        pf[p].y = r0[(long long)(2 * p + 1) * a.ld];
+      }
+    } else {
+#pragma unroll
+      for (int p = 0; p < NP; ++p) {
+        int la = rf.at(2 * p) - a.in_row0;
+        int lb = rf.at(2 * p + 1) - a.in_row0;
+        la = la < 0 ? 0 : (la > last_in ? last_in : la);
+        lb = lb < 0 ? 0 : (lb > last_in ? last_in : lb);
+        pf[p].x = a.in[(long long)la * a.ld + cx];
+        pf[p].y = a.in[(long long)lb * a.ld + cx];
+      }
+    }
+    rf.advance(ROWS);
+  };
+  auto epilogue = [&](int yyb) {
+    if (!owns) return;
+    [&]<int... I>(std::integer_sequence<int, I...>) {
+      (([&] {
+         if (flag) {
+           const int y0 = yyb - C::delay(I);
+           const bool dense = I == 0 && a.dense0;
+           const long long off0 = (long long)(y0 - a.out_row0) * a.ld + x;
+           if (y0 >= ys && y0 + ROWS <= ye && !dense) {
+             bool any = false;
+#pragma unroll
+             for (int r = 0; r < ROWS; ++r) any = any || hit[I][r];
+             if (any) {
+#pragma unroll
+               for (int r = 0; r < ROWS; ++r)
+                 if (hit[I][r]) {
+                   a.mask[off0 + (long long)r * a.ld] = 1;
+                   if (a.when != nullptr) a.when[off0 + (long long)r * a.ld] = (uint8_t)a.widx[I];
+                 }
+             }
+           } else {
+#pragma unroll
+             for (int r = 0; r < ROWS; ++r) {
+               const int y = y0 + r;
+               if (y >= ys && y < ye) {
+                 const long long off = off0 + (long long)r * a.ld;
+                 if (dense) {
+                   a.mask[off] = hit[I][r] ? 1 : 0;
+                   if (a.when != nullptr) a.when[off] = hit[I][r] ? (uint8_t)a.widx[I] : (uint8_t)0;
+                 } else if (hit[I][r]) {
+                   a.mask[off] = 1;
+                   if (a.when != nullptr) a.when[off] = (uint8_t)a.widx[I];
+                 }
+               }
+             }
+           }
+         }
+       }()), ...);
+    }(std::make_integer_sequence<int, NW>{});
+    const int yob = yyb - S;
+    if (yob >= ys) {
+      const long long off0 = (long long)(yob - a.out_row0) * a.ld + x;
+      if (yob + ROWS <= ye) {
+        if (a.nt) {
+#pragma unroll
+          for (int r = 0; r < ROWS; ++r) __builtin_nontemporal_store(outv[r], &a.out[off0 + (long long)r * a.ld]);
+        } else {
+#pragma unroll
+          for (int r = 0; r < ROWS; ++r) a.out[off0 + (long long)r * a.ld] = outv[r];
+        }
+      } else {
+#pragma unroll
+        for (int r = 0; r < ROWS; ++r)
+          if (yob + r < ye) smrf_store_out(&a.out[off0 + (long long)r * a.ld], outv[r], a.nt);
+      }
+    }
+  };
+
+  const bool scan = a.nan_flag != nullptr;
+  bool seen_nan = false;
+  prefetch();
+  for (int yy0 = ystart; yy0 < ye + S; yy0 += ROWS) {
+    T2 cur[NP];
+#pragma unroll
+    for (int p = 0; p < NP; ++p) cur[p] = pf[p];
+    if (scan) {
+#pragma unroll
+      for (int p = 0; p < NP; ++p) seen_nan = seen_nan || cur[p].x != cur[p].x || cur[p].y != cur[p].y;
+    }
+    if (yy0 > ystart) epilogue(yy0 - ROWS);
+    if (yy0 + ROWS < ye + S) prefetch();
+    T2 ecur[NP];
+#pragma unroll
+    for (int p = 0; p < NP; ++p) ecur[p] = cur[p];
+    [&]<int... I>(std::integer_sequence<int, I...>) {
+      (([&] {
+         constexpr int R = C::radius(I), KQ = C::kq(I), LAG = C::lag(I), WB = C::WB;
+         T2* const bufE = L;
+         T2* const bufD = L + C::BUF;
+         T lastv[ROWS];
+#pragma unroll
+         for (int r = 0; r < ROWS; ++r) {
+           const int e = r - LAG + KQ * ROWS, slot = e / ROWS, w = e % ROWS;
+           const T2 src = slot < KQ ? dq[I][slot < KQ ? slot : 0][w / 2] : cur[w / 2];
+           lastv[r] = (w & 1) ? src.y : src.x;
+         }
+#pragma unroll
+         for (int sl = 0; sl + 1 < KQ; ++sl)
+#pragma unroll
+           for (int p = 0; p < NP; ++p) dq[I][sl][p] = dq[I][sl + 1][p];
+#pragma unroll
+         for (int p = 0; p < NP; ++p) dq[I][KQ - 1][p] = cur[p];
+         if constexpr (C::cross(I)) {
+#pragma unroll
+           for (int p = 0; p < NP; ++p)
+             lds_write2((unsigned)(size_t)(__attribute__((address_space(3))) void*)(bufE + p * WB + 1 + tid), ecur[p]);
+           lds_wait<0>();
+           __syncthreads();
+           chain_cross_stage<T, NP, WB>(bufE, tid, xc[I], ecur);
+#pragma unroll
+           for (int p = 0; p < NP; ++p) cur[p] = ecur[p];
+         } else {
+#pragma unroll
+           for (int p = 0; p < NP; ++p)
+             lds_write2((unsigned)(size_t)(__attribute__((address_space(3))) void*)(bufE + p * WB + R + tid), cur[p]);
+           lds_wait<0>();
+           __syncthreads();
+           chain_stage<T, R, false, NP, WB>(bufE, tid, accE[I], cur);
+           if constexpr (C::cross(I + 1)) {
+#pragma unroll
+             for (int p = 0; p < NP; ++p) ecur[p] = cur[p];
+           }
+         }
+#pragma unroll
+         for (int p = 0; p < NP; ++p)
+           lds_write2((unsigned)(size_t)(__attribute__((address_space(3))) void*)(bufD + p * WB + R + tid), cur[p]);
+         lds_wait<0>();
+         __syncthreads();
+         chain_stage<T, R, true, NP, WB>(bufD, tid, accD[I], cur);
+#pragma unroll
+         for (int r = 0; r < ROWS; ++r) {
+           const T opened = (r & 1) ? cur[r / 2].y : cur[r / 2].x;
+           const T diff = lastv[r] - opened;
+           if constexpr (sizeof(T) == 4) hit[I][r] = diff > thr_lo[I];
+           else hit[I][r] = (double)diff > a.thr[I];
+         }
+       }()), ...);
+    }(std::make_integer_sequence<int, NW>{});
+#pragma unroll
+    for (int r = 0; r < ROWS; ++r) outv[r] = (r & 1) ? cur[r / 2].y : cur[r / 2].x;
+  }
+  {
+    const int nb = (ye + S - ystart + ROWS - 1) / ROWS;
+    epilogue(ystart + (nb - 1) * ROWS);
+  }
+  if (scan && seen_nan) atomicOr(a.nan_flag, 1u);
diff --git a/neilpy_amd/csrc/core.hip b/neilpy_amd/csrc/core.hip
--- a/neilpy_amd/csrc/core.hip
+++ b/neilpy_amd/csrc/core.hip
@@ -29,6 +29,7 @@
   s.ring_debug = env_int("SMRF_RING_DEBUG", 0);
   s.ero_inc = env_int("SMRF_ERO_INC", 1);
   s.dil_cross = env_int("SMRF_DIL_CROSS", 1);
+  s.small_cross = env_int("SMRF_SMALL_CROSS", 1);
   return s;
 }
 std::atomic<const SmrfSwitches*> g_sw{new SmrfSwitches(read_switches())};
diff --git a/neilpy_amd/csrc/morph.hip b/neilpy_amd/csrc/morph.hip
--- a/neilpy_amd/csrc/morph.hip
+++ b/neilpy_amd/csrc/morph.hip
@@ -6,6 +6,7 @@
 
 #include "smrf_common.h"
 #include "morph_chain.h"
+#include "smrf_small_cross.h"
 
 namespace {
 
@@ -259,6 +260,7 @@
 }
 
 thread_local std::vector<uint8_t> g_ero_inc_taken;
+thread_local std::vector<uint8_t> g_small_cross_taken;
 
 template <typename T>
 int progressive_filter_api(const T* Z, int rows, int cols, const int32_t* windows, const double* thr, int nwin,
@@ -280,24 +282,29 @@
     if (when) SMRF_HIP_CHECK(hipMemsetAsync(when, 0, plane, stream));
   }
   const SmrfSwitches& sw = smrf_sw();
-  SmrfPfRules rules{(int)sizeof(T), sw.fused, sw.chain, sw.ero_inc, impl, nan_aware > 0, 0, sw.dil_cross};
+  SmrfPfRules rules{(int)sizeof(T), sw.fused, sw.chain, sw.ero_inc, impl, nan_aware > 0, 0, sw.dil_cross, sw.small_cross};
   std::vector<int32_t> plan_buf((size_t)2 * nwin);
   int32_t* const route = plan_buf.data();
   int32_t* const pattern = route + nwin;
   g_ero_inc_taken.assign((size_t)nwin, 0);
-  std::vector<uint8_t> fold((size_t)nwin, 0);
+  std::vector<uint8_t> fold((size_t)nwin, 0), small((size_t)nwin, 0);
   std::vector<SmrfPfStep> steps((size_t)2 * nwin);
   int nsteps = 0;
   auto make_plan = [&](int with_nan) {
     rules.nan_aware = with_nan;
     smrf_pf_route(rules, windows, nwin, rows, (long long)plane, route, g_ero_inc_taken.data(), pattern);
     smrf_pf_fold(rules, windows, route, g_ero_inc_taken.data(), nwin, fold.data());
-    nsteps = smrf_pf_steps(windows, route, g_ero_inc_taken.data(), fold.data(), pattern, nwin, steps.data());
+    smrf_pf_small_cross(rules, windows, route, nwin, rows, (long long)plane, small.data());
+    nsteps = smrf_pf_steps(windows, route, g_ero_inc_taken.data(), fold.data(), pattern, nwin, steps.data(), small.data());
+    g_small_cross_taken.assign((size_t)nwin, 0);
+    for (int s = 0; s < nsteps; ++s)
+      if (steps[(size_t)s].kind == kPfStepChainCross)
+        for (int k = 0; k < steps[(size_t)s].len; ++k) g_small_cross_taken[(size_t)(steps[(size_t)s].win + k)] = (uint8_t)(k + 1);
   };
   make_plan(nan_aware > 0);
   unsigned* d_nan = nullptr;
   if (nan_aware < 0) {
-    if (nsteps > 0 && steps[0].kind == kPfStepChain && sw.nan_ride != 0) {
+    if (nsteps > 0 && (steps[0].kind == kPfStepChain || steps[0].kind == kPfStepChainCross) && sw.nan_ride != 0) {
       d_nan = reinterpret_cast<unsigned*>(E);
       SMRF_HIP_CHECK(hipMemsetAsync(d_nan, 0, sizeof(unsigned), stream));
       nan_aware = 0;
@@ -335,13 +342,24 @@
     const int i = st.win, r = windows[i];
     T* const dst = P[st.dst];
     switch (st.kind) {
-      case kPfStepChain: {
+      case kPfStepChain:
+      case kPfStepChainCross: {
         ChainArgs<T> c{};
         c.in = at(st.src); c.out = dst; c.mask = mask; c.when = when;
         for (int k = 0; k < st.len; ++k) { c.thr[k] = thr[i + k]; c.widx[k] = i + k; }
         c.dense0 = st.dense;
         c.nan_flag = d_nan;
-        if (int rc = chain_launch(st.pattern, c, rows, cols, cols, 0, rows, 0, rows, stream)) return rc;
+        if (st.kind == kPfStepChainCross) {
+          if constexpr (sizeof(T) == 4) {
+            set_band(c, rows, cols, cols, 0, rows, 0, rows);
+            c.seg = sw.ring_seg;
+            if (int rc = smrf_chain_cross_f32(st.pattern, c, stream)) return rc;
+          } else {
+            return smrf_fail(SMRF_E_HIP, "internal: no cross-stage chain at this dtype");
+          }
+        } else if (int rc = chain_launch(st.pattern, c, rows, cols, cols, 0, rows, 0, rows, stream)) {
+          return rc;
+        }
         if (d_nan) {
           unsigned h = 0;
           SMRF_HIP_CHECK(hipMemcpyAsync(&h, d_nan, sizeof(h), hipMemcpyDeviceToHost, stream));
@@ -471,6 +489,31 @@
   return chain_flag_api<double>(d_last, d_opened, d_mask, d_when_dropped, h_radii, h_thresholds, h_window_index, n_windows,
                                 img_rows, cols, ld, in_row0, in_rows, out_row0, out_rows, stream);
 }
+int smrf_pf_small_cross_windows(uint8_t* h_taken, int n) {
+  if (!h_taken || n < 0) return smrf_fail(SMRF_E_ARG, "null h_taken");
+  const int have = (int)g_small_cross_taken.size();
+  for (int i = 0; i < n; ++i) h_taken[i] = i < have ? g_small_cross_taken[(size_t)i] : 0;
+  return have;
+}
+int smrf_pf_small_cross_plan(int elem_size, const int32_t* h_windows, int n, int rows, int64_t cells, int nan_aware, int impl, int band,
+                             uint8_t* h_small) {
+  if (n < 0 || (n > 0 && (!h_windows || !h_small))) return smrf_fail(SMRF_E_ARG, "null pointer");
+  if ((elem_size != 4 && elem_size != 8) || rows < 1 || cells < 0 || band < 0 || band > 2)
+    return smrf_fail(SMRF_E_ARG, "bad plan question (element size %d, %d rows, band %d)", elem_size, rows, band);
+  for (int i = 0; i < n; ++i)
+    if (h_windows[i] < 0) return smrf_fail(SMRF_E_ARG, "negative window %d", h_windows[i]);
+  const SmrfSwitches& sw = smrf_sw();
+  const SmrfPfRules rules{elem_size, sw.fused, sw.chain, sw.ero_inc, impl, nan_aware != 0, band, sw.dil_cross, sw.small_cross};
+  std::vector<int32_t> route((size_t)n);
+  std::vector<uint8_t> inc((size_t)n), small((size_t)n);
+  smrf_pf_route(rules, h_windows, n, rows, (long long)cells, route.data(), inc.data());
+  smrf_pf_small_cross(rules, h_windows, route.data(), n, rows, (long long)cells, small.data());
+  for (int i = 0, k = 0; i < n; ++i) {
+    k = small[(size_t)i] == 0 ? 0 : small[(size_t)i] == kPfSmallMember ? k + 1 : 1;
+    h_small[i] = (uint8_t)k;
+  }
+  return SMRF_OK;
+}
 int smrf_pf_ero_inc_windows(uint8_t* h_taken, int n) {
   if (!h_taken || n < 0) return smrf_fail(SMRF_E_ARG, "null h_taken");
   const int have = (int)g_ero_inc_taken.size();
diff --git a/neilpy_amd/csrc/morph_chain.h b/neilpy_amd/csrc/morph_chain.h
--- a/neilpy_amd/csrc/morph_chain.h
+++ b/neilpy_amd/csrc/morph_chain.h
@@ -21,6 +21,7 @@
 
 SMRF_HIDDEN int smrf_chain_f32(int pattern, const ChainArgs<float>& a, hipStream_t s);
 SMRF_HIDDEN int smrf_chain_f64(int pattern, const ChainArgs<double>& a, hipStream_t s);
+SMRF_HIDDEN int smrf_chain_cross_f32(int xpattern, const ChainArgs<float>& a, hipStream_t s);
 
 #ifndef SMRF_CHAIN_NP_ALL
 #define SMRF_CHAIN_NP_ALL 0
@@ -31,21 +32,46 @@
 
 namespace smrf {
 
-template <int NP_, int R0, int R1, int R2, int R3>
+template <int NP_, int R0, int R1, int R2, int R3, unsigned XM = 0>
 struct ChainCfg {
   static constexpr int NP = NP_, ROWS = 2 * NP_, TW = 256;
   static constexpr int NW = (R0 > 0) + (R1 > 0) + (R2 > 0) + (R3 > 0);
   static constexpr int radius(int i) { return i == 0 ? R0 : i == 1 ? R1 : i == 2 ? R2 : R3; }
   static constexpr int RM = R3 > 0 ? R3 : R2 > 0 ? R2 : R1 > 0 ? R1 : R0;
+  static constexpr bool cross(int i) { return ((XM >> i) & 1u) != 0; }
+  static constexpr int edelay(int i) {
+    int e = 0, o = 0;
+    for (int j = 0; j <= i; ++j) {
+      e = j > 0 && cross(j) ? e + 1 : o + radius(j);
+      o = e + radius(j);
+    }
+    return e;
+  }
   static constexpr int delay(int i) {
-    int d = 0;
-    for (int j = 0; j <= i; ++j) d += 2 * radius(j);
-    return d;
-  }
+    if constexpr (XM == 0) {
+      int d = 0;
+      for (int j = 0; j <= i; ++j) d += 2 * radius(j);
+      return d;
+    } else {
+      return edelay(i) + radius(i);
+    }
+  }
+  static constexpr int lag(int i) { return i == 0 ? delay(0) : delay(i) - delay(i - 1); }
   static constexpr int S = delay(NW - 1);
   static constexpr int TWO = TW - 2 * S;
-  static constexpr int kq(int i) { return (2 * radius(i) + ROWS - 1) / ROWS; }
-  static constexpr int KQM = (2 * RM + ROWS - 1) / ROWS;
+  static constexpr int kq(int i) { return (lag(i) + ROWS - 1) / ROWS; }
+  static constexpr int kqm() {
+    int m = 0;
+    for (int i = 0; i < NW; ++i) m = kq(i) > m ? kq(i) : m;
+    return m;
+  }
+  static constexpr int KQM = kqm();
+  static constexpr bool ordered() {
+    for (int i = 0; i < NW; ++i)
+      if (lag(i) < 1) return false;
+    return true;
+  }
+  static constexpr bool valid() { return (XM & 1u) == 0 && (XM >> NW) == 0 && ordered(); }
   static constexpr int WB = TW + 2 * RM;
   static constexpr int BUF = NP * WB;
   static constexpr int CELLS = 2 * BUF;
@@ -189,208 +215,66 @@
   }(std::make_integer_sequence<int, NP>{});
 }
 
+template <typename T, int NP, int WB>
+__device__ __forceinline__ void chain_cross_stage(typename Vec2<T>::type* const buf, const int tid, T (&carry)[3],
+                                                  typename Vec2<T>::type (&io)[NP]) {
+  using T2 = typename Vec2<T>::type;
+  constexpr int ROWS = 2 * NP;
+  const unsigned base = (unsigned)(size_t)(__attribute__((address_space(3))) void*)(buf + tid);
+  T2 lft[NP], rgt[NP];
+  [&]<int... P>(std::integer_sequence<int, P...>) {
+    ((lft[P] = lds_read2<(P * WB) * (int)sizeof(T2)>(base, T()), rgt[P] = lds_read2<(P * WB + 2) * (int)sizeof(T2)>(base, T())), ...);
+  }(std::make_integer_sequence<int, NP>{});
+  lds_wait<0>();
+  T own[ROWS + 2], hm[ROWS + 1];
+  own[0] = carry[0];
+  own[1] = carry[1];
+  hm[0] = carry[2];
+#pragma unroll
+  for (int p = 0; p < NP; ++p) {
+    own[2 * p + 2] = io[p].x;
+    own[2 * p + 3] = io[p].y;
+    hm[2 * p + 1] = op3<false>(io[p].x, lft[p].x, rgt[p].x);
+    hm[2 * p + 2] = op3<false>(io[p].y, lft[p].y, rgt[p].y);
+  }
+#pragma unroll
+  for (int p = 0; p < NP; ++p) {
+    io[p].x = op3<false>(own[2 * p], hm[2 * p], own[2 * p + 2]);
+    io[p].y = op3<false>(own[2 * p + 1], hm[2 * p + 1], own[2 * p + 3]);
+  }
+  carry[0] = own[ROWS];
+  carry[1] = own[ROWS + 1];
+  carry[2] = hm[ROWS];
+}
+
 template <typename T, int NP, int OCC, int R0, int R1, int R2, int R3>
 __global__ __launch_bounds__(256, OCC)
 void chain_kernel(const ChainArgs<T> a) {
   using C = ChainCfg<NP, R0, R1, R2, R3>;
-  using T2 = typename Vec2<T>::type;
-  constexpr int NW = C::NW, ROWS = C::ROWS, TW = C::TW, S = C::S, TWO = C::TWO, RM = C::RM, KQM = C::KQM;
-  static_assert(TWO >= 64, "chain too long for a 256-column strip");
-  extern __shared__ __attribute__((aligned(16))) unsigned char smrf_lds[];
-  T2* const L = reinterpret_cast<T2*>(smrf_lds);
-
-  const int tid = threadIdx.x;
-  const int xe0 = (int)blockIdx.x * TWO - S;
-  const int x = xe0 + tid;
-  const bool owns = tid >= S && tid < TW - S && x < a.cols;
-  const int cx = smrf_fold(x, a.cols);
-  const int ys = a.out_row0 + (int)blockIdx.y * a.seg;
-  const int ye = min(a.out_row0 + a.out_rows, ys + a.seg);
-  const int last_in = a.in_rows - 1;
-  const bool flag = a.mask != nullptr;
-  float thr_lo[NW];
-#pragma unroll
-  for (int i = 0; i < NW; ++i) thr_lo[i] = a.thr_lo[i];
-
-  T accE[NW][2 * RM], accD[NW][2 * RM];
-#pragma unroll
-  for (int i = 0; i < NW; ++i)
-#pragma unroll
-    for (int s = 0; s < 2 * RM; ++s) { accE[i][s] = ident<T>(false); accD[i][s] = ident<T>(true); }
-  T2 dq[NW][KQM][NP];
-#pragma unroll
-  for (int i = 0; i < NW; ++i)
-#pragma unroll
-    for (int s = 0; s < KQM; ++s)
-#pragma unroll
-      for (int p = 0; p < NP; ++p) { dq[i][s][p].x = T(0); dq[i][s][p].y = T(0); }
-  T2 pf[NP];
-  T outv[ROWS];
-  bool hit[NW][ROWS];
-#pragma unroll
-  for (int r = 0; r < ROWS; ++r) {
-    outv[r] = T(0);
-#pragma unroll
-    for (int i = 0; i < NW; ++i) hit[i][r] = false;
-  }
-
-  constexpr int DELTA = (ROWS - (2 * S) % ROWS) % ROWS;
-  const int ystart = ys - S - DELTA;
-  RowFold rf(ystart, a.img_rows);
-  auto prefetch = [&]() {
-    const int l0 = rf.p - a.in_row0;
-    if (rf.p + ROWS <= rf.n && l0 >= 0 && l0 + ROWS - 1 <= last_in) {
-      const T* r0 = a.in + (long long)l0 * a.ld + cx;
-#pragma unroll
-      for (int p = 0; p < NP; ++p) {
-        pf[p].x = r0[(long long)(2 * p) * a.ld];
-        pf[p].y = r0[(long long)(2 * p + 1) * a.ld];
-      }
-    } else {
-#pragma unroll
-      for (int p = 0; p < NP; ++p) {
-        int la = rf.at(2 * p) - a.in_row0;
-        int lb = rf.at(2 * p + 1) - a.in_row0;
-        la = la < 0 ? 0 : (la > last_in ? last_in : la);
-        lb = lb < 0 ? 0 : (lb > last_in ? last_in : lb);
-        pf[p].x = a.in[(long long)la * a.ld + cx];
-        pf[p].y = a.in[(long long)lb * a.ld + cx];
-      }
-    }
-    rf.advance(ROWS);
-  };
-  auto epilogue = [&](int yyb) {
-    if (!owns) return;
-    [&]<int... I>(std::integer_sequence<int, I...>) {
-      (([&] {
-         if (flag) {
-           const int y0 = yyb - C::delay(I);
-           const bool dense = I == 0 && a.dense0;
-           const long long off0 = (long long)(y0 - a.out_row0) * a.ld + x;
-           if (y0 >= ys && y0 + ROWS <= ye && !dense) {
-             bool any = false;
-#pragma unroll
-             for (int r = 0; r < ROWS; ++r) any = any || hit[I][r];
-             if (any) {
-#pragma unroll
-               for (int r = 0; r < ROWS; ++r)
-                 if (hit[I][r]) {
-                   a.mask[off0 + (long long)r * a.ld] = 1;
-                   if (a.when != nullptr) a.when[off0 + (long long)r * a.ld] = (uint8_t)a.widx[I];
-                 }
-             }
-           } else {
-#pragma unroll
-             for (int r = 0; r < ROWS; ++r) {
-               const int y = y0 + r;
-               if (y >= ys && y < ye) {
-                 const long long off = off0 + (long long)r * a.ld;
-                 if (dense) {
-                   a.mask[off] = hit[I][r] ? 1 : 0;
-                   if (a.when != nullptr) a.when[off] = hit[I][r] ? (uint8_t)a.widx[I] : (uint8_t)0;
-                 } else if (hit[I][r]) {
-                   a.mask[off] = 1;
-                   if (a.when != nullptr) a.when[off] = (uint8_t)a.widx[I];
-                 }
-               }
-             }
-           }
-         }
-       }()), ...);
-    }(std::make_integer_sequence<int, NW>{});
-    const int yob = yyb - S;
-    if (yob >= ys) {
-      const long long off0 = (long long)(yob - a.out_row0) * a.ld + x;
-      if (yob + ROWS <= ye) {
-        if (a.nt) {
-#pragma unroll
-          for (int r = 0; r < ROWS; ++r) __builtin_nontemporal_store(outv[r], &a.out[off0 + (long long)r * a.ld]);
-        } else {
-#pragma unroll
-          for (int r = 0; r < ROWS; ++r) a.out[off0 + (long long)r * a.ld] = outv[r];
-        }
-      } else {
-#pragma unroll
-        for (int r = 0; r < ROWS; ++r)
-          if (yob + r < ye) smrf_store_out(&a.out[off0 + (long long)r * a.ld], outv[r], a.nt);
-      }
-    }
-  };
-
-  const bool scan = a.nan_flag != nullptr;
-  bool seen_nan = false;
-  prefetch();
-  for (int yy0 = ystart; yy0 < ye + S; yy0 += ROWS) {
-    T2 cur[NP];
-#pragma unroll
-    for (int p = 0; p < NP; ++p) cur[p] = pf[p];
-    if (scan) {
-#pragma unroll
-      for (int p = 0; p < NP; ++p) seen_nan = seen_nan || cur[p].x != cur[p].x || cur[p].y != cur[p].y;
-    }
-    if (yy0 > ystart) epilogue(yy0 - ROWS);
-    if (yy0 + ROWS < ye + S) prefetch();
-    [&]<int... I>(std::integer_sequence<int, I...>) {
-      (([&] {
-         constexpr int R = C::radius(I), KQ = C::kq(I), WB = C::WB;
-         T2* const bufE = L;
-         T2* const bufD = L + C::BUF;
-         T lastv[ROWS];
-#pragma unroll
-         for (int r = 0; r < ROWS; ++r) {
-           const int e = r - 2 * R + KQ * ROWS, slot = e / ROWS, w = e % ROWS;
-           const T2 src = slot < KQ ? dq[I][slot < KQ ? slot : 0][w / 2] : cur[w / 2];
-           lastv[r] = (w & 1) ? src.y : src.x;
-         }
-#pragma unroll
-         for (int sl = 0; sl + 1 < KQ; ++sl)
-#pragma unroll
-           for (int p = 0; p < NP; ++p) dq[I][sl][p] = dq[I][sl + 1][p];
-#pragma unroll
-         for (int p = 0; p < NP; ++p) dq[I][KQ - 1][p] = cur[p];
-#pragma unroll
-         for (int p = 0; p < NP; ++p)
-           lds_write2((unsigned)(size_t)(__attribute__((address_space(3))) void*)(bufE + p * WB + R + tid), cur[p]);
-         lds_wait<0>();
-         __syncthreads();
-         chain_stage<T, R, false, NP, WB>(bufE, tid, accE[I], cur);
-#pragma unroll
-         for (int p = 0; p < NP; ++p)
-           lds_write2((unsigned)(size_t)(__attribute__((address_space(3))) void*)(bufD + p * WB + R + tid), cur[p]);
-         lds_wait<0>();
-         __syncthreads();
-         chain_stage<T, R, true, NP, WB>(bufD, tid, accD[I], cur);
-#pragma unroll
-         for (int r = 0; r < ROWS; ++r) {
-           const T opened = (r & 1) ? cur[r / 2].y : cur[r / 2].x;
-           const T diff = lastv[r] - opened;
-           if constexpr (sizeof(T) == 4) hit[I][r] = diff > thr_lo[I];
-           else hit[I][r] = (double)diff > a.thr[I];
-         }
-       }()), ...);
-    }(std::make_integer_sequence<int, NW>{});
-#pragma unroll
-    for (int r = 0; r < ROWS; ++r) outv[r] = (r & 1) ? cur[r / 2].y : cur[r / 2].x;
-  }
-  {
-    const int nb = (ye + S - ystart + ROWS - 1) / ROWS;
-    epilogue(ystart + (nb - 1) * ROWS);
-  }
-  if (scan && seen_nan) atomicOr(a.nan_flag, 1u);
-}
-
-template <typename T, int NP, int OCC, int R0, int R1, int R2, int R3>
+#include "chain_kernel_body.inc"
+}
+template <typename T, int NP, int OCC, unsigned XM, int R0, int R1, int R2, int R3>
+__global__ __launch_bounds__(256, OCC)
+void chain_cross_kernel(const ChainArgs<T> a) {
+  using C = ChainCfg<NP, R0, R1, R2, R3, XM>;
+#include "chain_kernel_body.inc"
+}
+
+template <typename T, int NP, int OCC, int R0, int R1, int R2, int R3, unsigned XM = 0>
 int chain_launch(const ChainArgs<T>& a_in, hipStream_t stream) {
-  using C = ChainCfg<NP, R0, R1, R2, R3>;
+  using C = ChainCfg<NP, R0, R1, R2, R3, XM>;
   using T2 = typename Vec2<T>::type;
   constexpr size_t LDS = (size_t)C::CELLS * sizeof(T2);
-  constexpr auto kern = chain_kernel<T, NP, OCC, R0, R1, R2, R3>;
+  constexpr auto kern = [] {
+    if constexpr (XM == 0) return chain_kernel<T, NP, OCC, R0, R1, R2, R3>;
+    else return chain_cross_kernel<T, NP, OCC, XM, R0, R1, R2, R3>;
+  }();
   int resident;
   bool first;
   if (int rc = smrf_resident<kern>(C::TW, LDS, resident, first)) return rc;
   if (first && smrf_sw().ring_debug)
-    fprintf(stderr, "smrf chain: R=%d,%d,%d,%d %s NP=%d LDS=%zu, %d workgroups/CU resident\n", R0, R1, R2, R3,
-            sizeof(T) == 4 ? "f32" : "f64", NP, LDS, resident);
+    fprintf(stderr, "smrf chain: R=%d,%d,%d,%d cross=%u %s NP=%d LDS=%zu TWO=%d, %d workgroups/CU resident\n", R0, R1, R2, R3, XM,
+            sizeof(T) == 4 ? "f32" : "f64", NP, LDS, C::TWO, resident);
   ChainArgs<T> a = a_in;
   const int strips = (a.cols + C::TWO - 1) / C::TWO;
   a.seg = smrf_seg_len(a.out_rows, strips, resident, smrf_sw().chain_rounds, 2 * C::S, C::ROWS, std::max(32, 4 * C::S),
diff --git a/neilpy_amd/csrc/pf_route.h b/neilpy_amd/csrc/pf_route.h
--- a/neilpy_amd/csrc/pf_route.h
+++ b/neilpy_amd/csrc/pf_route.h
@@ -39,6 +39,28 @@
   return s;
 }
 
+struct SmrfCrossPattern { int n; int r[4]; unsigned cross; int halo; long long min_cells; };
+constexpr SmrfCrossPattern kCrossPatterns[] = {{3, {5, 6, 7, 0}, 6u, 14, kLarge}, {2, {6, 7, 0, 0}, 2u, 14, kLarge}, {3, {1, 2, 3, 0}, 2u, 10, kLarge}};
+constexpr int kNCrossPatterns = (int)(sizeof(kCrossPatterns) / sizeof(kCrossPatterns[0]));
+namespace smrf {
+#include "small_cross_adopt.inc"
+}
+static_assert(sizeof(smrf::kSmallCrossAdoptF32) / sizeof(smrf::kSmallCrossAdoptF32[0]) == kNCrossPatterns, "one entry per row of kCrossPatterns");
+constexpr int smrf_cross_halo(const SmrfCrossPattern& p) {
+  int e = 0, o = 0;
+  for (int j = 0; j < p.n; ++j) {
+    e = ((p.cross >> j) & 1u) ? e + 1 : o + p.r[j];
+    o = e + p.r[j];
+  }
+  return o;
+}
+constexpr bool smrf_cross_halos_hold() {
+  for (int p = 0; p < kNCrossPatterns; ++p)
+    if (smrf_cross_halo(kCrossPatterns[p]) != kCrossPatterns[p].halo) return false;
+  return true;
+}
+static_assert(smrf_cross_halos_hold(), "kCrossPatterns: halo");
+
 #ifndef SMRF_FUSED_MAX_RADIUS
 #define SMRF_FUSED_MAX_RADIUS 14
 #endif
@@ -80,6 +102,7 @@
   int nan_aware;
   int band;
   int dil_cross;
+  int small_cross;
 };
 
 inline void smrf_pf_route(const SmrfPfRules& k, const int32_t* windows, int n, int rows, long long cells, int32_t* route,
@@ -130,19 +153,47 @@
 }
 inline bool smrf_pf_runs_inc(const uint8_t* ero_inc, const uint8_t* fold, int i) { return ero_inc[i] != 0 && fold[i] == kPfFoldNone; }
 
-constexpr int kPfStepChain = 0, kPfStepFused = 1, kPfStepErode = 2, kPfStepIncErode = 3, kPfStepDilate = 4, kPfStepDilateCross = 5;
+constexpr uint8_t kPfSmallMember = 255;
+inline void smrf_pf_small_cross(const SmrfPfRules& k, const int32_t* windows, const int32_t* route, int n, int rows, long long cells,
+                                uint8_t* small) {
+  const bool ok = k.small_cross != 0 && !k.band && !k.nan_aware && k.elem_size == 4 && (k.impl == kPfImplAuto || k.impl == kPfImplRing) &&
+                  k.fused != 0 && k.chain != 0;
+  for (int i = 0; i < n; ++i) small[i] = 0;
+  for (int i = 0; ok && i < n;) {
+    int len = 0;
+    for (int p = 0; p < kNCrossPatterns && !len; ++p) {
+      const SmrfCrossPattern& c = kCrossPatterns[p];
+      if (c.n > n - i || c.halo >= rows) continue;
+      if (k.small_cross != 2 && (!smrf::kSmallCrossAdoptF32[p] || cells < c.min_cells)) continue;
+      bool match = route[i] == kPfRouteChain && (i + c.n == n || route[i + c.n] <= kPfRouteChain);
+      for (int j = 0; j < c.n && match; ++j) match = windows[i + j] == c.r[j] && route[i + j] >= kPfRouteChain;
+      if (!match) continue;
+      small[i] = (uint8_t)(p + 1);
+      for (int j = 1; j < c.n; ++j) small[i + j] = kPfSmallMember;
+      len = c.n;
+    }
+    i += len ? len : 1;
+  }
+}
+
+constexpr int kPfStepChain = 0, kPfStepFused = 1, kPfStepErode = 2, kPfStepIncErode = 3, kPfStepDilate = 4, kPfStepDilateCross = 5,
+              kPfStepChainCross = 6;
 constexpr int kPfPlaneZ = -1, kPfPlaneNone = -2;
 struct SmrfPfStep { int kind, win, len, src, aux, dst, dense, closes, pattern; };
 
 inline int smrf_pf_steps(const int32_t* windows, const int32_t* route, const uint8_t* ero_inc, const uint8_t* fold,
-                         const int32_t* pattern, int n, SmrfPfStep* steps) {
+                         const int32_t* pattern, int n, SmrfPfStep* steps, const uint8_t* small = nullptr) {
   (void)windows;
   int pe = 0, pl = kPfPlaneZ, m = 0;
   for (int i = 0; i < n;) {
     int po = 0;
     while (po == pe || po == pl) ++po;
     int len = 1;
-    if (route[i] == kPfRouteChain) {
+    if (small && small[i] != 0 && small[i] != kPfSmallMember) {
+      len = kCrossPatterns[small[i] - 1].n;
+      steps[m++] = {kPfStepChainCross, i, len, pl, kPfPlaneNone, po, i == 0, 1, small[i] - 1};
+      pl = po;
+    } else if (route[i] == kPfRouteChain) {
       len = smrf_chain_length(pattern[i]);
       steps[m++] = {kPfStepChain, i, len, pl, kPfPlaneNone, po, i == 0, 1, pattern[i]};
       pl = po;
diff --git a/neilpy_amd/csrc/small_cross_adopt.inc b/neilpy_amd/csrc/small_cross_adopt.inc
--- /dev/null
+++ b/neilpy_amd/csrc/small_cross_adopt.inc
@@ -0,0 +1,5 @@
+inline constexpr unsigned char kSmallCrossAdoptF32[3] = {
+    1,
+    1,
+    1,
+};
diff --git a/neilpy_amd/csrc/smrf_common.h b/neilpy_amd/csrc/smrf_common.h
--- a/neilpy_amd/csrc/smrf_common.h
+++ b/neilpy_amd/csrc/smrf_common.h
@@ -62,6 +62,7 @@
   int ring_debug;
   int ero_inc;
   int dil_cross;
+  int small_cross;
 };
 SMRF_HIDDEN const SmrfSwitches& smrf_sw();
 
```

After: 4386 (median of 5 runs). About the same (+0.2%).
